# jzebedee/deltaq

Hardware: AMD Instinct MI355X
Metric: MB of text suffix-sorted per second (bit-exact SA) (higher is better)
Workload: dtype u8 text / u64 keys / int32 SA; 1 GPU; 256 MiB uniform-random bytes per GPU (splitmix64 seed 0x5EED0003+rank), int32 SA; bytes_per_gpu=268435456, residency=text and SA resident in HBM, rounds_after_initial_sort=1

## Files before the change

deltaq_amd/csrc/dq_flags.h:

```cpp
#pragma once

#include <algorithm>
#include <cstdint>
#include <cstdlib>
#include <cstring>
#include <optional>
#include <string>

namespace dq {

struct Flags {
    bool debug = false;
    std::optional<int> trace;
    std::optional<int> hip_device;
    std::optional<int> numa_bind;
    std::optional<std::string> fault;
    std::optional<int> small_n;
    std::optional<int> no_many;
    std::optional<int> mid_many_min;
    std::optional<int> no_large_many;
    std::optional<int> large_many_min;
    std::optional<int> no_diff_many;
    std::optional<int> no_diff_mid_many;
    std::optional<int> diff_mid_many_min;
    std::optional<int> no_diff_large;
    std::optional<int> diff_large_min;
    std::optional<int> diff_large_table;
    std::optional<int> no_index_many;
    std::optional<int> index_many_min;
    std::optional<int> index_many_threads;
    std::optional<int> no_index_large;
    std::optional<int> index_large_min;
    std::optional<int> no_check_many;
    std::optional<int> no_bwt_many;
    std::optional<int> no_mtf_many;
    std::optional<int> no_huff_many;
    std::optional<int> mtf_short_max;
    std::optional<int> unbz2_one_start;
    bool no_list_buffers = false;
    bool text_copy = false;
    bool assume_doubled = false;
    bool no_twins = false;
    bool no_period_hint = false;
    std::optional<int> xcd_group;
    std::optional<int> packed;
    std::optional<int> key_bytes;
    std::optional<int> coded;
    std::optional<int> split;
    bool no_bucket = false;
    std::optional<int> bucket;
    std::optional<int> bucket_keybits;
    std::optional<int> bucket_ext;
    std::optional<int> bucket_tile;
    std::optional<int> bucket_slots;
    bool old_first_pass = false;
    bool no_fused_ties = false;
    std::optional<int> sparse;
    std::optional<int> binned_isa;
    bool no_binned_isa = false;
    std::optional<int> runs;
    bool no_small = false;
    bool no_wide_small = false;
    bool no_first_small = false;
    std::optional<int> mid_groups;
    bool no_l_shift = false;
    bool no_upd_words = false;
    std::optional<int> upd_bin;
    std::optional<int> upd_bin_min;
    std::optional<int> upd_window;
    std::optional<int> chain_steps;
    bool no_chain = false;
    bool force_rshift = false;
    std::optional<int> tail_max;
    std::optional<int> pair_chains;
    std::optional<int> pair_chains_min;
    std::optional<int> pair_maxg;
    std::optional<int> late_runs_min;
    bool no_late_runs = false;
    std::optional<int> run_period;
    bool search_wave = false;
    std::optional<int> search_ptab;
    bool no_wave_windows = false;
    bool no_poll = false;
    bool no_second_stage = false;
    std::optional<int> win_min;
    std::optional<int> win_second;
    std::optional<int> walk_on;
    bool no_resume = false;
    std::optional<int> scan_device;
    std::optional<int> scan_groups;
    std::optional<int> scan_groups_cap;
    std::optional<int> scan_chains;
    std::optional<int64_t> scan_min_seg;
    std::optional<int64_t> scan_extra;
    std::optional<int64_t> scan_lane_budget;
    std::optional<int> scan_poll_sleep;
    std::optional<int> scan_spin_log2;
    std::optional<int> scan_slow_group;
    std::optional<int> scan_par_emit;
    std::optional<int64_t> frame_follow_min;
    bool frame_after = false;
};

inline Flags read_flags()
{
    auto on = [](const char *name) { return getenv(name) != nullptr; };
    auto num = [](const char *name, int lo = INT32_MIN, int hi = INT32_MAX) -> std::optional<int> {
        const char *v = getenv(name);
        if (!v) return std::nullopt;
        return std::max(lo, std::min(hi, atoi(v)));
    };
    auto num64 = [](const char *name, int64_t lo) -> std::optional<int64_t> {
        const char *v = getenv(name);
        if (!v) return std::nullopt;
        return std::max<int64_t>(lo, atoll(v));
    };
    Flags f;
    const char *gate = getenv("DQ_DEBUG_FLAGS");
    f.debug = gate && atoi(gate) != 0;
    f.trace = num("DQ_TRACE");
    f.hip_device = num("DQ_HIP_DEVICE");
    f.numa_bind = num("DQ_NUMA_BIND");
    if (!f.debug) return f;

    if (const char *v = getenv("DQ_FAULT")) f.fault = v;
    f.small_n = num("DQ_SMALL_N", 0);
    f.no_many = num("DQ_NO_MANY", 0, 15);
    f.mid_many_min = num("DQ_MID_MANY_MIN", 1);
    f.no_large_many = num("DQ_NO_LARGE_MANY", 0, 1);
    f.large_many_min = num("DQ_LARGE_MANY_MIN", 1);
    f.no_diff_many = num("DQ_NO_DIFF_MANY", 0, 1);
    f.no_diff_mid_many = num("DQ_NO_DIFF_MID_MANY", 0, 1);
    f.diff_mid_many_min = num("DQ_DIFF_MID_MANY_MIN", 1);
    f.no_diff_large = num("DQ_NO_DIFF_LARGE", 0, 1);
    f.diff_large_min = num("DQ_DIFF_LARGE_MIN", 1);
    f.diff_large_table = num("DQ_DIFF_LARGE_TABLE", 0, 1);
    f.no_index_many = num("DQ_NO_INDEX_MANY", 0, 1);
    f.index_many_min = num("DQ_INDEX_MANY_MIN", 1);
    f.index_many_threads = num("DQ_INDEX_MANY_THREADS");
    f.no_index_large = num("DQ_NO_INDEX_LARGE", 0, 1);
    f.index_large_min = num("DQ_INDEX_LARGE_MIN", 1);
    f.no_check_many = num("DQ_NO_CHECK_MANY", 0, 1);
    f.no_bwt_many = num("DQ_NO_BWT_MANY", 0, 1);
    f.no_mtf_many = num("DQ_NO_MTF_MANY", 0, 1);
    f.no_huff_many = num("DQ_NO_HUFF_MANY", 0, 1);
    f.mtf_short_max = num("DQ_MTF_SHORT_MAX", 0);
    f.unbz2_one_start = num("DQ_UNBZ2_ONE_START", 0, 1);
    f.no_list_buffers = on("DQ_NO_LIST_BUFFERS");
    f.text_copy = on("DQ_TEXT_COPY");
    f.assume_doubled = on("DQ_ASSUME_DOUBLED");
    f.no_twins = on("DQ_NO_TWINS");
    f.no_period_hint = on("DQ_NO_PERIOD_HINT");

    f.xcd_group = num("DQ_XCD_GROUP", 0, 64);
    f.packed = num("DQ_PACKED");
    f.key_bytes = num("DQ_KEY_BYTES", 1, 8);
    f.coded = num("DQ_CODED");
    f.split = num("DQ_SPLIT");
    f.no_bucket = on("DQ_NO_BUCKET");
    f.bucket = num("DQ_BUCKET");
    f.bucket_keybits = num("DQ_BUCKET_KEYBITS");
    f.bucket_ext = num("DQ_BUCKET_EXT");
    f.bucket_tile = num("DQ_BUCKET_TILE", 0, 1);
    f.bucket_slots = num("DQ_BUCKET_SLOTS", 0, 1);
    f.old_first_pass = on("DQ_OLD_FIRST_PASS");
    f.no_fused_ties = on("DQ_NO_FUSED_TIES");
    f.sparse = num("DQ_SPARSE");
    f.binned_isa = num("DQ_BINNED_ISA");
    f.no_binned_isa = on("DQ_NO_BINNED_ISA");
    f.runs = num("DQ_RUNS");

    f.no_small = on("DQ_NO_SMALL");
    f.no_wide_small = on("DQ_NO_WIDE_SMALL");
    f.no_first_small = on("DQ_NO_FIRST_SMALL");
    f.mid_groups = num("DQ_MID_GROUPS");
    f.no_l_shift = on("DQ_NO_L_SHIFT");
    f.no_upd_words = on("DQ_NO_UPD_WORDS");
    f.upd_bin = num("DQ_UPD_BIN", 0, 2);
    f.upd_bin_min = num("DQ_UPD_BIN_MIN", 1);
    f.upd_window = num("DQ_UPD_WINDOW");
    f.chain_steps = num("DQ_CHAIN_STEPS");
    f.no_chain = on("DQ_NO_CHAIN");
    f.force_rshift = on("DQ_FORCE_RSHIFT");

    f.tail_max = num("DQ_TAIL_MAX", 0);
    f.pair_chains = num("DQ_PAIR_CHAINS");
    f.pair_chains_min = num("DQ_PAIR_CHAINS_MIN", 1);
    f.pair_maxg = num("DQ_PAIR_MAXG", 2);
    f.late_runs_min = num("DQ_LATE_RUNS_MIN", 1);
    f.no_late_runs = on("DQ_NO_LATE_RUNS");
    f.run_period = num("DQ_RUN_PERIOD", 1);

    f.search_wave = on("DQ_SEARCH_WAVE");
    f.search_ptab = num("DQ_SEARCH_PTAB");
    f.no_wave_windows = on("DQ_NO_WAVE_WINDOWS");
    f.no_poll = on("DQ_NO_POLL");
    f.no_second_stage = on("DQ_NO_SECOND_STAGE");
    f.win_min = num("DQ_WIN_MIN", 16);
    f.win_second = num("DQ_WIN_SECOND", 16);
    f.walk_on = num("DQ_WALK_ON");
    f.no_resume = on("DQ_NO_RESUME");

    f.scan_device = num("DQ_SCAN_DEVICE");
    f.scan_groups = num("DQ_SCAN_GROUPS", 8);
    f.scan_groups_cap = num("DQ_SCAN_GROUPS_CAP", 0);
    f.scan_chains = num("DQ_SCAN_CHAINS", 1);
    f.scan_min_seg = num64("DQ_SCAN_MIN_SEG", 64);
    f.scan_extra = num64("DQ_SCAN_EXTRA", 1);
    f.scan_lane_budget = num64("DQ_SCAN_LANE_BUDGET", 1);
    f.scan_poll_sleep = num("DQ_SCAN_POLL_SLEEP", 1, 32);
    f.scan_spin_log2 = num("DQ_SCAN_SPIN_LOG2", 1, 24);
    f.scan_slow_group = num("DQ_SCAN_SLOW_GROUP", 0, 255);
    f.scan_par_emit = num("DQ_SCAN_PAR_EMIT");
    f.frame_follow_min = num64("DQ_FRAME_FOLLOW_MIN", INT64_MIN);
    f.frame_after = on("DQ_FRAME_AFTER");
    return f;
}

struct FaultPlan {
    int alloc_at = 0, hip_at = 0;
    int alloc_seen = 0, hip_seen = 0;
    bool spin = false;
};
inline thread_local FaultPlan t_fault;

inline FaultPlan parse_fault(const std::optional<std::string> &spec)
{
    FaultPlan p;
    if (!spec) return p;
    const char *f = spec->c_str();
    if (strncmp(f, "alloc:", 6) == 0) p.alloc_at = std::max(1, atoi(f + 6));
    else if (strncmp(f, "hip:", 4) == 0) p.hip_at = std::max(1, atoi(f + 4));
    else if (strcmp(f, "spin") == 0) p.spin = true;
    return p;
}

struct FlagState {
    Flags snap;
    int depth = 0;
};
inline thread_local FlagState t_flags;

struct EnvScope {
    EnvScope()
    {
        if (t_flags.depth++ != 0) return;
        t_flags.snap = read_flags();
        t_fault = parse_fault(t_flags.snap.fault);
    }
    explicit EnvScope(const Flags &adopt)
    {
        if (t_flags.depth++ == 0) t_flags.snap = adopt;
    }
    ~EnvScope() { if (--t_flags.depth == 0) t_fault = FaultPlan{}; }
    EnvScope(const EnvScope &) = delete;
    EnvScope &operator=(const EnvScope &) = delete;
};

inline const Flags &flags()
{
    if (t_flags.depth == 0) t_flags.snap = read_flags();
    return t_flags.snap;
}

template <typename Fn>
auto with_flags(Fn fn)
{
    return [snap = flags(), fn = std::move(fn)](auto &&...args) mutable {
        EnvScope scope(snap);
        return fn(std::forward<decltype(args)>(args)...);
    };
}

}
```

deltaq_amd/csrc/dq_round0.h:

```cpp
#pragma once
#include "dq_sort_passes.h"
#include "dq_alpha_code.h"
#include "dq_ties.h"
#include "dq_bucket_sort.h"
#include "dq_xcd_rank.h"
#include "dq_slot_rank.h"

namespace dq {
namespace {

constexpr int64_t kSgShortList = 1 << 20;
inline int mid_group_cap(int64_t list_len)
{
    if (const std::optional<int> g = flags().mid_groups) {
        return *g >= 1024 ? 1024 : *g >= 512 ? 512 : *g >= 256 ? 256 : 0;
    }
    return list_len >= kSgShortList ? 512 : 1024;
}
inline bool small_round_usable(int64_t n, int64_t mm, bool third_list_buffer)
{
    const Flags &F = flags();
    return !F.no_small && n < (1ll << 32) && (mm * 2 <= n || (third_list_buffer && !F.no_wide_small));
}

template <typename Fn>
int with_bool(bool on, Fn fn)
{
    return on ? fn(std::true_type{}) : fn(std::false_type{});
}

constexpr int kXcdHistAt = kRadixSize + 16;

template <typename IdxT>
struct Round0Out {
    uint64_t *Kr[2] = {nullptr, nullptr};
    IdxT *Vr[2] = {nullptr, nullptr};
    int64_t m = 0, h = 0;
    int rbits = 0;
    bool dense_built = false;
    bool fin_done = false;
    int64_t fin_cap = 0, fin_left = 0;
    bool shallow_ties = false, keys_ready = false, list_ungrouped = false;
    const uint32_t *first_rank32 = nullptr;
    RunPlan runs;
};

template <typename IdxT>
struct Round0 {
    DeviceCtx &c;
    hipStream_t st;
    Workspace<IdxT> &w;
    int64_t n;
    IdxT *d_sa;
    Launcher &L;
    const uint8_t *text_src;
    int period_hint;
    Round0Out<IdxT> &o;

    static constexpr int64_t wb = (int64_t)sizeof(IdxT);
    TextStats s;
    KeyPlan k;
    int ib = 0;
    bool coded = false;
    uint64_t *K[2] = {w.K0, w.K1};
    IdxT *V[2] = {nullptr, nullptr};

    const uint64_t *text64() const { return reinterpret_cast<const uint64_t *>(w.text); }
    int64_t tie_words() const { return (n + 63) / 64; }

    int digit_tables(int kb, bool coded_keys)
    {
        if (coded_keys) {
            const int hblocks = (int)std::min<int64_t>(kHistBlocks, ((n >> 2) + kHistThreads - 1) / kHistThreads + 1);
            DQ_TRY(L.begin(DQ_K_RADIX_HIST, n, n));
            HIP_TRY(hipMemsetAsync(w.hist_partial, 0, (size_t)kMaxPasses * kRadixSize * 8, st));
            hipLaunchKernelGGL(text_coded_hist_kernel, dim3(hblocks), dim3(kHistThreads), 0, st,
                               reinterpret_cast<const uint32_t *>(w.text), n, (const uint16_t *)w.codetab,
                               reinterpret_cast<unsigned long long *>(w.hist_partial));
            hipLaunchKernelGGL(radix_hist_scan_kernel, dim3(kMaxPasses), dim3(kHistScanThreads), 0, st,
                               (const unsigned long long *)w.hist_partial, w.digit_offset);
            HIP_TRY(hipGetLastError());
            return L.end();
        }
        hipLaunchKernelGGL(text_digit_offsets_kernel, dim3(kb), dim3(kBlock), 0, st,
                           (const int64_t *)w.bytehist, (const uint8_t *)w.text, n, kb, w.digit_offset);
        HIP_TRY(hipGetLastError());
        return DQ_OK;
    }

    int prepare()
    {
        int blocks = (int)std::min<int64_t>(1024, ((n >> 4) + kBlock - 1) / kBlock + 1);
        unsigned long long *xcd_hist = n >= kRound0MinN ? reinterpret_cast<unsigned long long *>(w.bytehist + kXcdHistAt) : nullptr;
        if (xcd_hist) blocks = (blocks + kXcds - 1) / kXcds * kXcds;
        HIP_TRY(hipMemsetAsync(w.bytehist, 0, (size_t)(kXcdHistAt + (xcd_hist ? kXcds * kRadixSize : 0)) * 8, L.st));
        LAUNCH(L, DQ_K_TEXT_HIST, n, n,
               hipLaunchKernelGGL(text_hist_kernel, dim3(blocks + 1), dim3(kBlock), 0, L.st,
                                  text_src ? text_src : (const uint8_t *)w.text, n, reinterpret_cast<unsigned long long *>(w.bytehist),
                                  reinterpret_cast<unsigned long long *>(w.bytehist + 256), text_src ? w.text : (uint8_t *)nullptr,
                                  xcd_hist));
        HIP_TRY(hipMemcpyAsync(c.pinned, w.bytehist, (256 + 10) * 8, hipMemcpyDeviceToHost, L.st));
        HIP_TRY(hipEventRecord(c.readback, L.st));
        constexpr int kEarlyPasses = 3;
        DQ_TRY(prepare_status<IdxT>(L, w, n, kEarlyPasses));
        if (n >= kRound0MinN) HIP_TRY(hipMemsetAsync(w.Vb, 0, (size_t)(tie_words() + 1) * 8, L.st));
        HIP_TRY(hipEventSynchronize(c.readback));
        const Flags &F = flags();
        s = TextStats(c.pinned, n);
        ib = s.ib;
        k = choose_key_bytes(s, F);
        DQ_TRY(prepare_status<IdxT>(L, w, n, k.kb, kEarlyPasses));
        bool hist_deferred = false;
        if (coded_keys_tried(s, F, k)) {
            AlphaCode code;
            if (build_alpha_code(s.hist, &code) && (code.avg_len <= kCodedMaxAvgLen || F.coded)) {
                uint16_t *stage = reinterpret_cast<uint16_t *>(c.pinned + 512);
                memcpy(stage, code.tab, sizeof(code.tab));
                HIP_TRY(hipMemcpyAsync(w.codetab, stage, sizeof(code.tab), hipMemcpyHostToDevice, L.st));
                coded = true;
                hist_deferred = split_round0_wanted(n, k, (int)wb, F);
                if (F.trace) fprintf(stderr, "[dq] coded round 0: %d symbols, %.2f bits per byte\n", code.sigma, code.avg_len);
            }
        }
        if (hist_deferred) return DQ_OK;
        return digit_tables(k.kb, coded);
    }

    int passes(int &cur, uint32_t *ebits = nullptr, uint64_t *seam_tab = nullptr)
    {
        const int kb = k.kb;
        if (k.packed) {
            DQ_TRY(rank_pass<IdxT, kTextPacked>(L, w, text64(), (const IdxT *)nullptr, K[1], (IdxT *)nullptr, n, 0, kb, ib));
            cur = 1;
            for (int p = 1; p < kb; ++p) {
                if (p == kb - 1 && ebits)
                    DQ_TRY(rank_pass<IdxT, kKeysLastTies>(L, w, K[cur], (const IdxT *)nullptr, (uint64_t *)nullptr, d_sa, n, p,
                                                          kb, ib, ebits, seam_tab));
                else if (p == kb - 1)
                    DQ_TRY(rank_pass<IdxT, kKeysLast>(L, w, K[cur], (const IdxT *)nullptr, K[cur ^ 1], d_sa, n, p, kb, ib));
                else
                    DQ_TRY(rank_pass<IdxT, kKeys>(L, w, K[cur], (const IdxT *)nullptr, K[cur ^ 1], (IdxT *)nullptr, n, p, kb, ib));
                cur ^= 1;
            }
            return DQ_OK;
        }
        DQ_TRY(with_bool(coded, [&](auto kCoded) -> int {
            return rank_pass<IdxT, kText, decltype(kCoded)::value>(L, w, text64(), (const IdxT *)nullptr, K[1], V[1], n, 0, kb);
        }));
        cur = 1;
        for (int p = 1; p < kb; ++p) {
            DQ_TRY(rank_pass<IdxT, kPairs>(L, w, K[cur], V[cur], K[cur ^ 1], V[cur ^ 1], n, p, kb));
            cur ^= 1;
        }
        return DQ_OK;
    }

    int collect_ties(uint32_t *ebits, const uint64_t *seam_tab, uint64_t *act_rank, bool *overflow, uint64_t *fin_rank,
                     bool seams = true, int64_t h_fin = -1)
    {
        using Cfg = RankCfg<IdxT, kKeysLastTies>;
        using CfgS = RankCfg<IdxT, kKeysLastTies, true>;
        const int64_t tile_keys = small_tiles(n) ? CfgS::kThreads * CfgS::kItems : Cfg::kThreads * Cfg::kItems;
        const int64_t ntiles = (n + tile_keys - 1) / tile_keys;
        const int pass = k.kb - 1;
        char *area = w.ctl_status + (size_t)pass * w.ctl_status_stride;
        const int64_t *dofs = w.digit_offset + pass * kRadixSize;
        TieCounters *ctr = reinterpret_cast<TieCounters *>(w.totals + 6);
        if (seams) {
            HIP_TRY(hipMemsetAsync(ctr, 0, sizeof(TieCounters), L.st));
            const unsigned sg = (unsigned)((ntiles * kRadixSize + kBlock - 1) / kBlock);
            DQ_TRY(with_status_word(n, [&](auto word) -> int {
                LAUNCH(L, DQ_K_TIE_SEAM, ntiles * kRadixSize, ntiles * kRadixSize * (16 + (int64_t)sizeof(uint64_t)),
                       hipLaunchKernelGGL(tie_seam_kernel<decltype(word)>, dim3(sg), dim3(kBlock), 0, L.st, seam_tab, ntiles, ib, dofs,
                                          reinterpret_cast<const decltype(word) *>(area + 256), ebits));
                return DQ_OK;
            }));
        }
        LAUNCH(L, DQ_K_TIE_COLLECT, n, n / 8,
               hipLaunchKernelGGL(tie_collect_kernel<IdxT>, dim3((unsigned)((tie_words() + kTieThreads - 1) / kTieThreads)),
                                  dim3(kTieThreads), 0, L.st, reinterpret_cast<const uint64_t *>(ebits), tie_words(), n, (const IdxT *)d_sa,
                                  act_rank, w.Va, ctr));
        unsigned long long *left_over = reinterpret_cast<unsigned long long *>(w.totals + 3);
        o.fin_cap = n / 8;
        LAUNCH(L, DQ_K_SMALL_FINISH, o.fin_cap, 0,
               hipLaunchKernelGGL((small_group_finish_kernel<IdxT, 8, 32>),
                                  dim3((unsigned)std::min<int64_t>((o.fin_cap + kFinishThreads - 1) / kFinishThreads, 256 * 16)),
                                  dim3(kFinishThreads), 0, L.st, (const uint64_t *)act_rank, (const IdxT *)w.Va, (const uint8_t *)w.text,
                                  o.fin_cap, n, h_fin >= 0 ? h_fin : (int64_t)k.kb, d_sa, fin_rank, w.Vb, left_over,
                                  (const unsigned long long *)&ctr->count));
        DQ_TRY(read_totals<IdxT>(L, c, w, 64, "radix look-back timed out (device spin bound hit)"));
        o.m = c.pinned[6];
        *overflow = c.pinned[7] != 0;
        if (*overflow && flags().trace) fprintf(stderr, "[dq] tie / bucket overflow flags: %lld\n", (long long)c.pinned[7]);
        o.fin_left = c.pinned[3];
        if (L.active && !c.pending.empty() && c.pending.back().cat == DQ_K_SMALL_FINISH) {
            const int64_t cnt = std::min<int64_t>(o.m, o.fin_cap);
            c.pending.back().elems = cnt;
            c.pending.back().bytes = cnt * (8 + wb + 64 + wb);
        }
        return DQ_OK;
    }

    int build_isa_binned(uint64_t *keys, uint64_t *P0, int kshift0)
    {
        const int64_t ntiles = (n + kSegFusedTile - 1) / kSegFusedTile;
        const size_t need = 256 + (size_t)3 * ntiles * 8;
        if (need > w.seg_status_bytes) return fail(DQ_ERR_HIP, "seg status buffer too small");
        HIP_TRY(hipMemsetAsync(w.seg_status, 0, need, st));
        const bool rank32_direct = sizeof(IdxT) == 4 && !o.runs.runs_wanted && mid_group_cap(n) > 0;
        const bool third = w.X != nullptr;
        uint32_t *list_rank = (small_round_usable(n, 0, third) && !flags().no_first_small)
                                  ? (rank32_direct ? w.RL : reinterpret_cast<uint32_t *>(w.Vb)) : nullptr;
        LAUNCH(L, DQ_K_SEG_FUSED, n, n * (8 + wb + 8),
               hipLaunchKernelGGL((seg_fused_kernel<IdxT, true, false, false, true>), dim3((unsigned)ntiles),
                                  dim3(kSegThreads), 0, st, (const uint64_t *)keys, (const IdxT *)d_sa, n, ib, kshift0,
                                  d_sa, w.ISA, P0, w.Va, reinterpret_cast<uint64_t *>(w.seg_status + 256), ntiles,
                                  reinterpret_cast<SegCtl *>(w.seg_status), w.totals, w.totals + 1, 0, list_rank, 0, spin_bound()));
        const int rc = read_totals<IdxT>(L, c, w, 16, "device look-back timed out (spin bound hit)");
        o.m = c.pinned[0];
        DQ_TRY(rc);
        DQ_TRY(isa_from_suffix_words<IdxT>(L, c, w, n, ib, k.kb, P0, keys));
        if (list_rank && o.m == 0) return DQ_OK;
        if (list_rank && small_round_usable(n, o.m, third) && rank32_direct) {
            o.first_rank32 = list_rank;
            return DQ_OK;
        }
        if (list_rank && small_round_usable(n, o.m, third)) {
            LAUNCH(L, DQ_K_KEY2_FROM_PAIRS, o.m, o.m * 12,
                   hipLaunchKernelGGL(widen_ranks_kernel, dim3(grid_for(o.m)), dim3(kBlock), 0, st,
                                      (const uint32_t *)list_rank, o.m, keys));
            return DQ_OK;
        }
        const bool with_key2 = !o.runs.runs_wanted;
        const int kbits = bit_length((uint64_t)(n - 1) + (uint64_t)k.kb);
        unsigned long long *cnt = reinterpret_cast<unsigned long long *>(w.totals + 3);
        HIP_TRY(hipMemsetAsync(cnt, 0, 8, st));
        const int64_t per = (int64_t)kPairThreads * kPairItems;
        LAUNCH(L, DQ_K_KEY2_FROM_PAIRS, n, n * 8 + o.m * (wb + 8 + wb),
               hipLaunchKernelGGL(key2_from_pairs_kernel<IdxT>, dim3((unsigned)((n + per - 1) / per)), dim3(kPairThreads),
                                  0, st, (const uint64_t *)P0, n, ib, (const IdxT *)w.ISA, (int64_t)k.kb, kbits, with_key2,
                                  keys, w.Va, cnt));
        o.keys_ready = with_key2;
        o.list_ungrouped = true;
        return DQ_OK;
    }

    int bucketed(bool *done)
    {
        *done = false;
        const Flags &F = flags();
        const BucketPlan b = plan_bucketed(s, F, k, coded, (int)wb);
        if (!b.applies) return DQ_OK;
        const int kb = k.kb, keybits = b.keybits, lowbits = b.lowbits;
        const SlotPlan sp = bucket_slots_fit(s, b, (int)wb);
        const FinishTiles ft = plan_finish_tiles(b, n, F, sp.fits);
        static_assert(sizeof(SlotRankCtl) <= (size_t)kHistBlocks * kMaxPasses * kRadixSize * 4, "the cursors live in the histogram scratch");
        const bool slots = bucket_slots_wanted(sp, ft, F) && (uint64_t)sp.words <= slot_span_words_of(w) &&
                           (size_t)(2 * kSlotBuckets + 5) * 4 <= finish_bounds_entries(n) * 8;
        uint32_t *slot_base = reinterpret_cast<uint32_t *>(w.bkt_bounds), *slot_out = slot_base + kSlotBuckets + 4;
        SlotRankCtl *sctl = reinterpret_cast<SlotRankCtl *>(w.hist_partial);
        const int first = slots ? 0 : 1;
        uint8_t *E[2] = {reinterpret_cast<uint8_t *>(w.Va), reinterpret_cast<uint8_t *>(w.Va) + align_up((size_t)n)};
        uint32_t *ebits = reinterpret_cast<uint32_t *>(w.Vb);
        TieCounters *ctr = reinterpret_cast<TieCounters *>(w.totals + 6);
        BucketFlags *bflags = reinterpret_cast<BucketFlags *>(&ctr->overflow);
        hipLaunchKernelGGL(text_digit_offsets_kernel, dim3(b.bbytes), dim3(kBlock), 0, st,
                           (const int64_t *)w.bytehist, (const uint8_t *)w.text, n, b.bbytes, w.digit_offset,
                           b.xcd_pass ? (const int64_t *)(w.bytehist + kXcdHistAt) : nullptr, b.xcd_pass ? w.xcd_offset : nullptr);
        HIP_TRY(hipGetLastError());
        if (slots) {
            if (F.trace)
                fprintf(stderr, "[dq] second pass into bucket slots: %d x %d slots of %lld words (n=%lld)\n", sp.first, sp.second,
                        (long long)b.X, (long long)n);
            HIP_TRY(hipMemsetAsync(sctl, 0, sizeof(SlotRankCtl), st));
            hipLaunchKernelGGL(slot_plan_kernel, dim3(kRadixSize + 1), dim3(kBlock), 0, st, (const int64_t *)w.bytehist, b.X, slot_base);
            HIP_TRY(hipGetLastError());
        }
        if (c.ncu <= 0) {
            int v = 0;
            c.ncu = hipDeviceGetAttribute(&v, hipDeviceAttributeMultiprocessorCount, c.dev) == hipSuccess && v > 0 ? v : 256;
        }
        if (b.xcd_pass) {
            if (F.trace) fprintf(stderr, "[dq] XCD-local first pass (n=%lld, eighths of %lld)\n", (long long)n, (long long)xcd_eighth(n));
            if (sizeof(XcdRankCtl) > w.ctl_status_stride) return fail(DQ_ERR_HIP, "status buffer too small");
            LAUNCH(L, DQ_K_RADIX_RANK, n, n * (1 + 8),
                   hipLaunchKernelGGL(xcd_text_rank_kernel, dim3((unsigned)std::min<int64_t>(c.ncu, (n + kXcdTileN - 1) / kXcdTileN)),
                                      dim3(kXcdRankThreads), 0, st, reinterpret_cast<const uint32_t *>(w.text), K[first], n,
                                      ib + lowbits, keybits, ib, (const int64_t *)w.xcd_offset,
                                      reinterpret_cast<XcdRankCtl *>(w.ctl_status)));
        } else {
            DQ_TRY(b.ext ? rank_pass_ext<IdxT, kTextPackedExt>(L, w, text64(), (const uint8_t *)nullptr, K[1], E[1], n, 0, ib, ib + lowbits, keybits)
                       : rank_pass<IdxT, kTextPacked>(L, w, text64(), (const IdxT *)nullptr, K[first], (IdxT *)nullptr, n, 0, kb, ib,
                                                      nullptr, nullptr, ib + lowbits, keybits));
        }
        if (slots) {
            const int groups = resident_groups(&c.slot_rank_groups, (const void *)slot_rank_kernel, kSlotRankThreads, c.dev);
            LAUNCH(L, DQ_K_RADIX_RANK, n, n * 16,
                   hipLaunchKernelGGL(slot_rank_kernel, dim3((unsigned)std::min<int64_t>(groups, (n + kSlotTileN - 1) / kSlotTileN)),
                                      dim3(kSlotRankThreads), 0, st, (const uint64_t *)K[0], K[1], n, ib + lowbits + 8, ib + lowbits,
                                      (const int64_t *)w.digit_offset, (const uint32_t *)slot_base, sctl, bflags));
        }
        for (int p = 1; p < b.bbytes && !slots; ++p) {
            DQ_TRY(b.ext ? rank_pass_ext<IdxT, kKeysExt>(L, w, K[p & 1], E[p & 1], K[(p & 1) ^ 1], E[(p & 1) ^ 1], n, p, ib, ib + lowbits + 8 * p, keybits)
                       : rank_pass<IdxT, kKeys>(L, w, K[p & 1], (const IdxT *)nullptr, K[(p & 1) ^ 1], (IdxT *)nullptr, n, p, kb, ib,
                                                nullptr, nullptr, ib + lowbits + 8 * p, keybits));
        }
        uint64_t *Ks = slots ? K[1] : K[b.bbytes & 1], *Kfree = slots ? K[0] : K[(b.bbytes & 1) ^ 1];
        const uint8_t *Es = b.ext ? E[b.bbytes & 1] : nullptr;
        if (F.trace)
            fprintf(stderr, "[dq] bucket finish: %s geometry, %lld tiles of up to %lld words cut every %lld %s (n=%lld)\n", ft.fine ? "fine" : "coarse",
                    (long long)ft.ntiles, (long long)ft.cap, (long long)(ft.by_id ? ft.g : ft.Cf), ft.by_id ? "buckets" : "words", (long long)n);
        if ((size_t)ft.ntiles + 1 > finish_bounds_entries(n)) return fail(DQ_ERR_HIP, "tile bounds buffer too small");
        if (slots) {
            LAUNCH(L, DQ_K_BUCKET_SORT, ft.ntiles, ft.ntiles * 16,
                   hipLaunchKernelGGL(slot_out_kernel, dim3(1), dim3(kSlotOutThreads), 0, st, sctl->cursor, (uint32_t)b.X, slot_out, bflags));
            auto kernel = bucket_sort_kernel<IdxT, false, BktFine, true>;
            const int groups = resident_groups(&c.bkt_slot_groups[sizeof(IdxT) == 8], (const void *)kernel, BktFine::threads, c.dev);
            LAUNCH(L, DQ_K_BUCKET_SORT, n, n * (8 + wb) + n / 8,
                   hipLaunchKernelGGL(kernel, dim3((unsigned)std::min<int64_t>(ft.ntiles, groups)), dim3(BktFine::threads), 0, st,
                                      (const uint64_t *)Ks, ib, lowbits, (const int64_t *)nullptr, ft.ntiles, d_sa, ebits, bflags,
                                      (const uint8_t *)nullptr, (const uint32_t *)slot_base, (const uint32_t *)sctl->cursor, (const uint32_t *)slot_out));
        } else if (ft.by_id) {
            const int64_t nbuckets = (int64_t)1 << (8 * b.bbytes);
            LAUNCH(L, DQ_K_BUCKET_SORT, ft.ntiles, ft.ntiles * 16 * 8,
                   hipLaunchKernelGGL(bucket_bounds_by_id_kernel, dim3((unsigned)((nbuckets + 1 + kBlock - 1) / kBlock)), dim3(kBlock), 0,
                                      st, (const uint64_t *)Ks, n, ib + lowbits, ft.g, b.X, nbuckets, ft.ntiles, w.bkt_bounds, bflags));
        } else {
            LAUNCH(L, DQ_K_BUCKET_SORT, ft.ntiles, ft.ntiles * 16 * 8,
                   hipLaunchKernelGGL(bucket_bounds_kernel, dim3((unsigned)((ft.ntiles + 1 + kBlock - 1) / kBlock)), dim3(kBlock), 0,
                                      st, (const uint64_t *)Ks, n, ib + lowbits, ft.Cf, b.X, ft.ntiles, w.bkt_bounds, bflags));
        }
        auto finish = [&](auto kExt, auto geometry) -> int {
            using G = decltype(geometry);
            auto kernel = bucket_sort_kernel<IdxT, decltype(kExt)::value, G>;
            const int groups = resident_groups(&c.bkt_groups[ft.fine][b.ext][sizeof(IdxT) == 8], (const void *)kernel, G::threads, c.dev);
            LAUNCH(L, DQ_K_BUCKET_SORT, n, n * ((b.ext ? 9 : 8) + wb) + n / 8,
                   hipLaunchKernelGGL(kernel, dim3((unsigned)std::min<int64_t>(ft.ntiles, groups)), dim3(G::threads), 0, st,
                                      (const uint64_t *)Ks, ib, lowbits, (const int64_t *)w.bkt_bounds, ft.ntiles, d_sa, ebits, bflags, Es,
                                      (const uint32_t *)nullptr, (const uint32_t *)nullptr, (const uint32_t *)nullptr));
            return DQ_OK;
        };
        if (slots) {
        } else if (ft.fine) {
            DQ_TRY(finish(std::false_type{}, BktFine{}));
        } else {
            DQ_TRY(with_bool(b.ext, [&](auto kExt) -> int { return finish(kExt, BktCoarse{}); }));
        }
        if (b.ext && F.trace) fprintf(stderr, "[dq] bucketed round 0 with %d + 8 key bits per suffix (n=%lld)\n", keybits, (long long)n);
        bool overflow = false;
        DQ_TRY(collect_ties(ebits, nullptr, Kfree, &overflow, Ks, false, b.hb));
        if (overflow) {
            if (F.trace) fprintf(stderr, "[dq] bucketed round 0 gave up (n=%lld): plain digit passes\n", (long long)n);
            DQ_TRY(prepare_status<IdxT>(L, w, n, kMaxPasses));
            HIP_TRY(hipMemsetAsync(w.Vb, 0, (size_t)(tie_words() + 1) * 8, st));
            HIP_TRY(hipMemsetAsync(w.totals, 0, 64, st));
            o.m = 0; o.fin_cap = 0; o.fin_left = 0;
            return digit_tables(kb, false);
        }
        o.fin_done = o.m <= o.fin_cap;
        o.Kr[0] = Kfree; o.Kr[1] = Ks;
        o.h = b.hb;
        o.shallow_ties = true;
        *done = true;
        return DQ_OK;
    }

    int split(bool *done)
    {
        *done = false;
        if constexpr (sizeof(IdxT) != 4) {
            return DQ_OK;
        } else {
            if (!w.sp_top || !w.X || !w.RL) return DQ_OK;
            const int64_t cap = std::min<int64_t>(kFinCap, (n + 2) / (kSplitBuckets / 2));
            if (cap < 2) return DQ_OK;
            const uint32_t *t32 = reinterpret_cast<const uint32_t *>(w.text);
            const uint16_t *ctab = (const uint16_t *)w.codetab;
            uint64_t *Ks[2] = {K[0], w.X};
            IdxT *Vs[2] = {w.Vb, w.Xs};
            const int64_t ovf_cap = (n / 2) & ~(int64_t)1;
            uint64_t *ovf_k[2] = {reinterpret_cast<uint64_t *>(w.ISA), K[0]};
            IdxT *ovf_v[2] = {reinterpret_cast<IdxT *>(w.RL), w.Vb};
            const Flags &F = flags();
            const bool dbg = F.trace.value_or(0) >= 2;
            auto phase = [&](const char *what) -> int {
                if (!dbg) return DQ_OK;
                HIP_TRY(hipStreamSynchronize(st));
                fprintf(stderr, "[dq] split round 0: %s done\n", what);
                return DQ_OK;
            };
            const unsigned sgrid = (unsigned)((kSplitSample + kBlock - 1) / kBlock);
            DQ_TRY(with_bool(coded, [&](auto kCoded) -> int {
                LAUNCH(L, DQ_K_SPLIT_AUX, kSplitSample, kSplitSample * ((coded ? 20 : 12) + 8),
                       hipLaunchKernelGGL(sample_keys_kernel<decltype(kCoded)::value>, dim3(sgrid), dim3(kBlock), 0, st, t32, n, ctab, kSplitSample, Ks[0]));
                return DQ_OK;
            }));
            DQ_TRY(phase("sample"));
            int scur = 0;
            DQ_TRY(onesweep_sort_pairs<IdxT>(L, w, Ks, Vs, kSplitSample, 64, scur));
            DQ_TRY(phase("sample sort"));
            HIP_TRY(hipMemsetAsync(w.sp_ctl, 0, sizeof(SplitCtl), st));
            hipLaunchKernelGGL(sample_heavy_kernel, dim3(sgrid), dim3(kBlock), 0, st, (const uint64_t *)Ks[scur], &w.sp_ctl->ovf_count);
            HIP_TRY(hipGetLastError());
            HIP_TRY(hipMemcpyAsync(c.pinned, w.sp_ctl, sizeof(SplitCtl), hipMemcpyDeviceToHost, st));
            HIP_TRY(hipStreamSynchronize(st));
            const int64_t heavy = c.pinned[0];
            if (F.trace)
                fprintf(stderr, "[dq] sample-sort round 0: %.1f %% of the sampled keys are copies of keys too heavy for a bucket%s\n",
                        100.0 * (double)heavy / (double)kSplitSample, heavy * 5 > 2 * kSplitSample ? " -- the digit passes instead" : "");
            if (heavy * 5 > 2 * kSplitSample && F.split.value_or(0) < 2) return DQ_OK;
            HIP_TRY(hipMemsetAsync(w.sp_cursor_b, 0, (size_t)kSplitBuckets * 8, st));
            HIP_TRY(hipMemsetAsync(w.sp_ctl, 0, sizeof(SplitCtl), st));
            const int64_t n_main = n & ~(int64_t)1;
            uint64_t *spill_k = reinterpret_cast<uint64_t *>(d_sa);
            IdxT *spill_v = d_sa + (n / 2 + 1);
            if (n / 8 + 1025 * (int64_t)kSplitTop + 1024 > n / 4) return DQ_OK;
            LAUNCH(L, DQ_K_SPLIT_AUX, kSplitBuckets, (int64_t)kSplitBuckets * 16,
                   hipLaunchKernelGGL(make_splitters_kernel, dim3(kSplitBuckets / kBlock), dim3(kBlock), 0, st, (const uint64_t *)Ks[scur], w.sp_top, w.sp_sub,
                                      w.sp_low, w.sp_pure);
                   hipLaunchKernelGGL(split_estimate_kernel, dim3(1), dim3(kSplitTop), 0, st, (const uint64_t *)Ks[scur], (const uint64_t *)w.sp_top, n, w.sp_off,
                                      w.sp_cursor_a));
            DQ_TRY(phase("splitters, region estimates"));
            const unsigned grid_a = (unsigned)((n + kSplitTileA - 1) / kSplitTileA);
            DQ_TRY(with_bool(coded, [&](auto kCoded) -> int {
                LAUNCH(L, DQ_K_SPLIT_PASS, n, n * (1 + 8 + wb),
                       hipLaunchKernelGGL((split_pass_kernel<IdxT, true, decltype(kCoded)::value>), dim3(grid_a), dim3(kSplitThreads), 0, st, text64(), (const IdxT *)nullptr,
                                          (const uint64_t *)nullptr, (const IdxT *)nullptr, (int64_t)0, n, (const uint64_t *)w.sp_top, w.sp_cursor_a,
                                          (const int64_t *)w.sp_off, (const unsigned long long *)nullptr, (const uint32_t *)w.sp_tile_first, K[1], w.Va, spill_k, spill_v,
                                          n_main, (uint64_t *)nullptr, (IdxT *)nullptr, (int64_t)0, w.sp_ctl, ctab));
                return DQ_OK;
            }));
            DQ_TRY(phase("pass A"));
            const unsigned grid_b = (unsigned)(n / kSplitTileB + kSplitTop);
            LAUNCH(L, DQ_K_SPLIT_PASS, n, n * 2 * (8 + wb),
                   hipLaunchKernelGGL(split_plan_kernel, dim3(1), dim3(kSplitTop), 0, st, (const unsigned long long *)w.sp_cursor_a, (const int64_t *)w.sp_off, w.sp_cnt_a,
                                      w.sp_tile_first, w.sp_ctl);
                   hipLaunchKernelGGL((split_pass_kernel<IdxT, false, false>), dim3(grid_b), dim3(kSplitThreads), 0, st, (const uint64_t *)K[1], (const IdxT *)w.Va,
                                      (const uint64_t *)spill_k, (const IdxT *)spill_v, n_main, n, (const uint64_t *)w.sp_sub, w.sp_cursor_b, (const int64_t *)w.sp_off,
                                      (const unsigned long long *)w.sp_cnt_a, (const uint32_t *)w.sp_tile_first, Ks[0], Vs[0], Ks[1], Vs[1],
                                      cap, ovf_k[0], ovf_v[0], ovf_cap, w.sp_ctl, ctab, (const uint8_t *)w.sp_pure));
            DQ_TRY(phase("pass B"));
            LAUNCH(L, DQ_K_SPLIT_AUX, kSplitBuckets, (int64_t)kSplitBuckets * 36,
                   hipLaunchKernelGGL(bucket_sum_kernel, dim3(kScanBlocks), dim3(kScanThreads), 0, st, (const unsigned long long *)w.sp_cursor_b, cap,
                                      (const uint8_t *)w.sp_pure, w.sp_part);
                   hipLaunchKernelGGL(bucket_scan_kernel, dim3(kScanBlocks), dim3(kScanThreads), 0, st, (const unsigned long long *)w.sp_cursor_b, cap,
                                      (const uint8_t *)w.sp_pure, (const ScanPart *)w.sp_part, w.sp_out_base, w.sp_ovf_src, w.sp_ovf_dst, w.sp_ctl));
            DQ_TRY(phase("bucket scan"));
            const bool two = cap > kFinSmallCap;
            LAUNCH(L, DQ_K_SPLIT_FINISH, n, n * 2 * (8 + wb),
                   if (two || cap <= kFinSmallCap)
                       hipLaunchKernelGGL((bucket_finish_kernel<IdxT, 256, 4>), dim3(kSplitBuckets), dim3(256), 0, st, (const uint64_t *)Ks[0], (const IdxT *)Vs[0],
                                          (const uint64_t *)Ks[1], (const IdxT *)Vs[1], cap, (int64_t)0, (int64_t)kFinSmallCap, !two,
                                          (const unsigned long long *)w.sp_cursor_b, (const int64_t *)w.sp_out_base, K[1], d_sa, ovf_k[0], ovf_v[0], ovf_cap, w.sp_ctl, (const uint8_t *)w.sp_pure);
                   if (cap > kFinSmallCap)
                       hipLaunchKernelGGL((bucket_finish_kernel<IdxT, 256, 8>), dim3(kSplitBuckets), dim3(256), 0, st, (const uint64_t *)Ks[0], (const IdxT *)Vs[0],
                                          (const uint64_t *)Ks[1], (const IdxT *)Vs[1], cap, (int64_t)(two ? kFinSmallCap : 0), (int64_t)kFinCap, true,
                                          (const unsigned long long *)w.sp_cursor_b, (const int64_t *)w.sp_out_base, K[1], d_sa, ovf_k[0], ovf_v[0], ovf_cap, w.sp_ctl, (const uint8_t *)w.sp_pure));
            HIP_TRY(hipMemcpyAsync(c.pinned, w.sp_ctl, sizeof(SplitCtl), hipMemcpyDeviceToHost, st));
            HIP_TRY(hipStreamSynchronize(st));
            const int64_t ovf = c.pinned[0], ovf_buckets = c.pinned[1], npure = c.pinned[4];
            const bool abandon = c.pinned[3] != 0 || ovf + npure > ovf_cap;
            if (flags().trace)
                fprintf(stderr, "[dq] sample-sort round 0 (%s keys, %d buckets of <= %lld): %lld suffixes in %lld oversize buckets, %lld copies of heavy keys placed unsorted%s\n",
                        coded ? "coded" : "raw", kSplitBuckets, (long long)cap, (long long)ovf, (long long)ovf_buckets, (long long)npure,
                        abandon ? " -- overflow lists full, given up" : "");
            if (abandon) return DQ_OK;
            if (npure > 0) {
                LAUNCH(L, DQ_K_SPLIT_AUX, npure, npure * 2 * (8 + wb),
                       hipLaunchKernelGGL(pure_place_kernel<IdxT>, dim3((unsigned)((npure + kBlock - 1) / kBlock)), dim3(kBlock), 0, st, npure, ovf_cap,
                                          (const uint64_t *)ovf_k[0], (const IdxT *)ovf_v[0], (const int64_t *)w.sp_out_base, (const uint64_t *)w.sp_low, K[1], d_sa));
            }
            if (ovf > 0) {
                int xcur = 0;
                DQ_TRY(onesweep_sort_pairs<IdxT>(L, w, ovf_k, ovf_v, ovf, 64, xcur));
                LAUNCH(L, DQ_K_SPLIT_AUX, ovf, ovf * 2 * (8 + wb),
                       hipLaunchKernelGGL(overflow_place_kernel<IdxT>, dim3((unsigned)((ovf + kBlock - 1) / kBlock)), dim3(kBlock), 0, st, ovf, ovf_buckets,
                                          (const int64_t *)w.sp_ovf_src, (const int64_t *)w.sp_ovf_dst,
                                          (const uint64_t *)ovf_k[xcur], (const IdxT *)ovf_v[xcur], K[1], d_sa));
            }
            *done = true;
            return DQ_OK;
        }
    }

    int run()
    {
        const Flags &F = flags();
        int cur = 0;
        DQ_TRY(prepare());
        const int kb = k.kb;
        o.runs = plan_runs(s, F, (int)wb, period_hint);
        V[kb & 1] = d_sa;
        V[(kb & 1) ^ 1] = w.Va;
        o.Vr[0] = w.Va; o.Vr[1] = w.Vb;
        o.rbits = ib;
        o.h = kb;
        bool done = false;
        DQ_TRY(bucketed(&done));
        if (done) return DQ_OK;
        if (fused_ties_wanted(n, k, F)) {
            uint32_t *ebits = reinterpret_cast<uint32_t *>(w.Vb);
            uint64_t *seam_tab = reinterpret_cast<uint64_t *>(reinterpret_cast<char *>(w.Vb) +
                                                              align_up((size_t)(tie_words() + 1) * 8));
            DQ_TRY(passes(cur, ebits, seam_tab));
            bool overflow = false;
            DQ_TRY(collect_ties(ebits, seam_tab, K[cur], &overflow, K[cur ^ 1]));
            o.fin_done = !overflow && o.m <= o.fin_cap;
            if (!overflow) {
                o.Kr[0] = K[cur]; o.Kr[1] = K[cur ^ 1];
                return DQ_OK;
            }
            HIP_TRY(hipMemsetAsync(w.ctl_status + (size_t)(kb - 1) * w.ctl_status_stride, 0, w.ctl_status_stride, st));
            DQ_TRY(rank_pass<IdxT, kKeysLast>(L, w, K[cur ^ 1], (const IdxT *)nullptr, K[cur], d_sa, n, kb - 1, kb, ib));
        } else {
            bool split_done = false;
            const bool split_wanted = split_round0_wanted(n, k, (int)wb, F);
            if (split_wanted && (!o.runs.runs_wanted || F.split)) {
                DQ_TRY(split(&split_done));
            }
            if (split_wanted && !split_done) {
                DQ_TRY(digit_tables(kb, coded));
                DQ_TRY(prepare_status<IdxT>(L, w, n, kb));
            }
            if (split_done) {
                cur = 1;
            } else {
                DQ_TRY(passes(cur));
            }
        }
        const int kshift0 = k.packed ? ib : 0;
        const DenseGuess guess = dense_guess(n, k);
        int64_t tied_pairs = 0;
        if (guess == DenseGuess::kTakeSample) {
            HIP_TRY(hipMemsetAsync(w.totals + 2, 0, 8, st));
            hipLaunchKernelGGL(sample_ties_kernel, dim3(kTieSamples / kBlock), dim3(kBlock), 0, st,
                               (const uint64_t *)K[cur], n, kshift0, kTieSamples, w.totals + 2);
            HIP_TRY(hipGetLastError());
            HIP_TRY(hipMemcpyAsync(c.pinned, w.totals + 2, 8, hipMemcpyDeviceToHost, st));
            HIP_TRY(hipStreamSynchronize(st));
            tied_pairs = c.pinned[0];
        }
        o.dense_built = predict_dense(guess, tied_pairs, F);
        if (o.dense_built && binned_isa_pays(n, F)) {
            o.Kr[0] = K[cur]; o.Kr[1] = K[cur ^ 1];
            return build_isa_binned(K[cur], K[cur ^ 1], kshift0);
        }
        o.Kr[0] = K[cur ^ 1]; o.Kr[1] = K[cur];
        return o.dense_built ? rebucket<IdxT, true, false, true>(L, c, w, K[cur], (const IdxT *)d_sa, n, 0, kshift0, d_sa, o.Kr[0], w.Va, &o.m)
                             : rebucket<IdxT, true, false, false>(L, c, w, K[cur], (const IdxT *)d_sa, n, 0, kshift0, d_sa, o.Kr[0], w.Va, &o.m);
    }
};

}
}
```

deltaq_amd/csrc/dq_round0_plan.h:

```cpp
#pragma once
#include <algorithm>
#include <cmath>
#include <cstddef>
#include <cstdint>

#include "dq_flags.h"

namespace dq {

constexpr int kKgramSamples = 1024;
constexpr int kBktCap = 12288;
constexpr int kBktCapFine = 6144;
constexpr int kSplitTop = 512;
constexpr int kSplitSub = 512;
constexpr int kSplitBuckets = kSplitTop * kSplitSub;
constexpr int kFinCap = 2048;
constexpr int64_t kSplitMinN = 5ll << 20;
constexpr int64_t kCodedMinN = 8ll << 20;
constexpr double kCodedMaxAvgLen = 5.8;
constexpr int kTieSamples = 4096;
constexpr int64_t kRound0MinN = 1 << 16;

inline int index_bits(int64_t n) { return n <= 1 ? 1 : 64 - __builtin_clzll((uint64_t)(n - 1)); }

struct TextStats {
    int64_t n = 0;
    int ib = 1;
    int64_t hist[256] = {};
    int64_t kgram[8] = {};
    bool long_run = false;
    int64_t run_chunks = 0;
    double h0 = 0;
    int sigma = 0;
    int64_t cmax = 0;

    TextStats() = default;
    TextStats(const int64_t *words, int64_t n_) : n(n_), ib(index_bits(n_)), long_run(words[256 + 8] != 0), run_chunks(words[256 + 9])
    {
        std::copy(words, words + 256, hist);
        std::copy(words + 256, words + 256 + 8, kgram);
        for (int b = 0; b < 256; ++b) {
            cmax = std::max(cmax, hist[b]);
            if (hist[b] > 0) { ++sigma; const double p = (double)hist[b] / (double)n; h0 -= p * std::log2(p); }
        }
    }
};

struct KeyPlan { int kb = 8; bool packed = false; };

inline KeyPlan choose_key_bytes(const TextStats &s, const Flags &F)
{
    const int64_t n = s.n;
    const double need = std::log2((double)std::max<int64_t>(n, 2)) + 10.0;
    int kb = 8;
    if (s.h0 >= 0.25) kb = std::min(8, std::max(3, (int)std::ceil(need / s.h0)));
    const int fit = (64 - s.ib) / 8;
    bool packed = fit >= 2 && (kb <= fit || (double)fit * s.h0 >= std::log2((double)std::max<int64_t>(n, 2)) + 3.0);
    if (n >= kKgramSamples * 8) {
        const int L = packed ? std::min(kb, fit) : kb;
        const int64_t C = s.kgram[std::max(L, 1) - 1];
        const double twins = (double)n * 2.0 * (double)C / ((double)kKgramSamples * (double)kKgramSamples);
        if (C >= kKgramSamples / 16 && twins > 0.25) { packed = false; kb = 8; }
    }
    if (F.packed) packed = *F.packed != 0 && fit >= 2;
    if (packed) kb = std::min(kb, fit);
    if (F.key_bytes) {
        kb = *F.key_bytes;
        if (kb > fit || kb < 2) packed = false;
    }
    return {kb, packed};
}

inline bool coded_keys_tried(const TextStats &s, const Flags &F, KeyPlan k)
{
    bool coded = !k.packed && k.kb == 8 && s.n >= kCodedMinN;
    if (coded) coded = s.h0 <= kCodedMaxAvgLen - 0.25 && (s.sigma <= 128 || s.n >= 2 * kCodedMinN);
    if (F.coded) coded = *F.coded != 0 && !k.packed && k.kb == 8 && s.n >= 64;
    return coded;
}

inline bool split_round0_wanted(int64_t n, KeyPlan k, int idx_bytes, const Flags &F)
{
    if (idx_bytes != 4 || k.packed || k.kb != 8 || n < kSplitMinN || n > (int64_t)kSplitBuckets * (kFinCap / 2)) return false;
    if (F.split) return *F.split != 0;
    if (F.key_bytes || F.no_bucket) return false;
    return n >= (64ll << 20);
}

struct BucketPlan {
    bool applies = false;
    int keybits = 0, bbytes = 0, lowbits = 0;
    int64_t X = 0, C = 0, ntiles = 0;
    bool ext = false;
    bool xcd_pass = false;
    int64_t hb = 0;
};

inline BucketPlan plan_bucketed(const TextStats &s, const Flags &F, KeyPlan k, bool coded, int idx_bytes)
{
    const int64_t n = s.n;
    const int ib = s.ib;
    BucketPlan p;
    if (coded) return p;
    if (F.no_bucket || F.no_fused_ties || F.sparse || F.key_bytes) return p;
    const bool forced = F.bucket.has_value();
    if (ib > 31 || n < kRound0MinN) return p;
    if (!forced && s.long_run) return p;
    int keybits = std::min(64 - ib, 36);
    if (F.bucket_keybits) keybits = std::max(17, std::min(keybits, *F.bucket_keybits));
    const double tied = (double)n * std::exp2(-(double)keybits * s.h0 / 8.0);
    if (!k.packed) {
        if (!forced && (k.kb >= 8 || tied > 0.3)) return p;
    }
    const double pm = (double)s.cmax / (double)n;
    int bbytes = 2;
    double est = (double)n * pm * pm;
    double need = est + 6.0 * std::sqrt(est) + 64.0;
    const bool force3 = forced && *F.bucket == 3;
    if (need > 5120 || (!forced && n < (12 << 20)) || force3) {
        if (keybits - 24 >= 8 && (forced || n >= (12 << 20))) {
            bbytes = 3;
            est *= pm;
            need = est + 6.0 * std::sqrt(est) + 64.0;
        }
        if (need > 5120 || (bbytes == 2 && !forced)) {
            if (!forced) return p;
            need = 5120;
        }
    }
    p.applies = true;
    p.keybits = keybits;
    p.bbytes = bbytes;
    p.X = std::min<int64_t>(((int64_t)need + 255) / 256 * 256, 5120);
    p.C = kBktCap - p.X;
    p.lowbits = keybits - 8 * bbytes;
    p.ntiles = (n + p.C - 1) / p.C;
    const bool room = (size_t)2 * (((size_t)n + 255) / 256 * 256) <= (size_t)(n + 2) * (size_t)idx_bytes;
    p.ext = keybits + 8 <= 56 && p.lowbits + 8 <= 18 && tied > 0.02 && room;
    if (F.bucket_ext) p.ext = *F.bucket_ext != 0 && keybits + 8 <= 56 && room;
    p.xcd_pass = !p.ext && !F.old_first_pass;
    p.hb = (keybits + (p.ext ? 8 : 0)) / 8;
    return p;
}

constexpr int64_t kBktFineMinN = 12ll << 20;
struct FinishTiles {
    bool fine = false;
    bool by_id = false;
    int64_t cap = 0;
    int64_t Cf = 0, g = 0;
    int64_t ntiles = 0;
};

inline FinishTiles plan_finish_tiles(const BucketPlan &b, int64_t n, const Flags &F, bool slots_fit = false)
{
    FinishTiles t;
    if (!b.applies) return t;
    const bool can = b.bbytes == 2 && !b.ext;
    t.fine = can && (F.bucket_tile ? *F.bucket_tile != 0 : !F.bucket.has_value() && n >= kBktFineMinN);
    t.cap = t.fine ? kBktCapFine : kBktCap;
    const int64_t Cf = t.cap - b.X;
    const bool force_by_id = t.fine && slots_fit && F.bucket_slots && *F.bucket_slots == 1;
    if (force_by_id) {
        t.by_id = true;
        t.g = 1;
        t.ntiles = (int64_t)1 << (8 * b.bbytes);
    } else if (Cf >= b.X) {
        t.Cf = Cf;
        t.ntiles = (n + Cf - 1) / Cf;
    } else {
        t.by_id = true;
        t.g = std::min<int64_t>(t.cap / b.X, 64);
        const int64_t nbuckets = (int64_t)1 << (8 * b.bbytes);
        t.ntiles = (nbuckets + t.g - 1) / t.g;
    }
    return t;
}

inline int64_t slot_span_words(int64_t n, int idx_bytes) { return (n + 2) * (int64_t)(8 + idx_bytes) / 8; }

struct SlotPlan {
    bool fits = false;
    int first = 0, second = 0;
    int64_t words = 0;
};

inline SlotPlan bucket_slots_fit(const TextStats &s, const BucketPlan &b, int idx_bytes)
{
    SlotPlan p;
    if (!b.applies || b.bbytes != 2 || b.ext) return p;
    p.first = s.sigma;
    p.second = s.sigma + (s.hist[0] == 0 ? 1 : 0);
    p.words = (int64_t)p.first * p.second * b.X;
    p.fits = p.words <= slot_span_words(s.n, idx_bytes) && p.words < ((int64_t)1 << 32);
    return p;
}

inline void slot_bases(const int64_t *hist , int64_t X, uint32_t *base )
{
    int ra[257], rb[257];
    ra[0] = rb[0] = 0;
    for (int d = 0; d < 256; ++d) {
        ra[d + 1] = ra[d] + (hist[d] > 0 ? 1 : 0);
        rb[d + 1] = rb[d] + (hist[d] > 0 || d == 0 ? 1 : 0);
    }
    for (int A = 0; A < 256; ++A)
        for (int B = 0; B < 256; ++B)
            base[A * 256 + B] = (uint32_t)(X * ((int64_t)ra[A] * rb[256] + (hist[A] > 0 ? rb[B] : 0)));
    base[65536] = (uint32_t)(X * ra[256] * rb[256]);
}

inline bool bucket_slots_wanted(const SlotPlan &p, const FinishTiles &t, const Flags &F)
{
    if (F.bucket_slots && *F.bucket_slots == 0) return false;
    return p.fits && t.fine && t.by_id && t.g == 1;
}

inline size_t finish_bounds_entries(int64_t n)
{
    const size_t by_words = (size_t)n / (kBktCapFine / 2) + 4;
    return n < kRound0MinN ? by_words : std::max<size_t>(by_words, 65536 + 4);
}

inline bool fused_ties_wanted(int64_t n, KeyPlan k, const Flags &F)
{
    return k.packed && k.kb >= 2 && n >= kRound0MinN && !F.no_fused_ties && !F.sparse;
}

enum class DenseGuess { kNeither, kGuessDense, kTakeSample };

inline DenseGuess dense_guess(int64_t n, KeyPlan k)
{
    if (n < kRound0MinN || k.packed || k.kb != 8) return DenseGuess::kNeither;
    return n < (8 << 20) ? DenseGuess::kGuessDense : DenseGuess::kTakeSample;
}

inline bool predict_dense(DenseGuess g, int64_t tied_pairs, const Flags &F)
{
    if (F.sparse) return *F.sparse == 0;
    return g == DenseGuess::kGuessDense || (g == DenseGuess::kTakeSample && tied_pairs * 12 > kTieSamples);
}

inline bool binned_isa_pays(int64_t n, const Flags &F)
{
    const bool pays = F.binned_isa ? *F.binned_isa != 0 : n > (32ll << 20);
    return pays && n >= kRound0MinN && 2 * index_bits(n) <= 63 && !F.no_binned_isa;
}

struct RunPlan {
    bool runs_wanted = false;
    bool long_run_seen = false;
    bool late_runs_possible = false;
};

inline RunPlan plan_runs(const TextStats &s, const Flags &F, int idx_bytes, int period_hint)
{
    RunPlan r;
    const bool can = idx_bytes == 4 && s.n >= kRound0MinN;
    r.long_run_seen = can && s.long_run;
    r.runs_wanted = (r.long_run_seen && s.run_chunks * 16 * 16 >= s.n) || (period_hint > 0 && can);
    r.late_runs_possible = can;
    if (F.runs) { r.runs_wanted = idx_bytes == 4 && *F.runs != 0; r.late_runs_possible = r.late_runs_possible && *F.runs != 0; }
    if (F.mid_groups) r.runs_wanted = r.runs_wanted && *F.mid_groups >= 256;
    return r;
}

}
```

deltaq_amd/csrc/dq_sa_kernels.h:

```cpp
#pragma once
#include "dq_runs.h"
#include "dq_device_utils.h"

namespace dq {

template <typename IdxT>
__global__ __launch_bounds__(kBlock) void gather_key2_kernel(uint64_t *__restrict__ comp,
                                                             const IdxT *__restrict__ suf,
                                                             const IdxT *__restrict__ ISA,
                                                             int64_t m, int64_t n, int64_t h, int kbits,
                                                             int rshift = 0,
                                                             const uint32_t *__restrict__ RL = nullptr ,
                                                             const uint8_t *__restrict__ text = nullptr, int run_order = 0)
{
    for (int64_t j = (int64_t)blockIdx.x * kBlock + threadIdx.x; j < m;
         j += (int64_t)gridDim.x * kBlock) {
        const int64_t s = (int64_t)suf[j];
        int64_t off = h;
        uint64_t k2 = 0;
        bool keyed = false;
        if (RL) {
            const uint32_t r = RL[s];
            if (run_order) { k2 = (int64_t)r >= h ? (uint64_t)run_order_key(text, n, s, r, run_order) : 0ull; keyed = true; }
            else if ((int64_t)r > h) off = (int64_t)r;
        }
        if (!keyed) {
            const int64_t q = s + off;
            k2 = q < n ? (uint64_t)((int64_t)ISA[q] + h) : (off > h ? 0ull : (uint64_t)(n - 1 - s));
        }
        comp[j] = ((comp[j] >> rshift) << kbits) | k2;
    }
}

static __global__ __launch_bounds__(kBlock) void keys_to_ranks_kernel(uint64_t *__restrict__ comp, int64_t m, int kbits)
{
    for (int64_t j = (int64_t)blockIdx.x * kBlock + threadIdx.x; j < m; j += (int64_t)gridDim.x * kBlock)
        comp[j] >>= kbits;
}

template <typename IdxT>
__global__ __launch_bounds__(kBlock) void gather_text_key_kernel(uint64_t *__restrict__ comp,
                                                                 const IdxT *__restrict__ suf,
                                                                 const uint8_t *__restrict__ text,
                                                                 int64_t m, int64_t n, int64_t h, int ebytes)
{
    const int kbits = 8 * ebytes + 3;
    for (int64_t j = (int64_t)blockIdx.x * kBlock + threadIdx.x; j < m;
         j += (int64_t)gridDim.x * kBlock) {
        const int64_t q = (int64_t)suf[j] + h;
        int64_t len = n - q;
        len = len < 0 ? 0 : (len > ebytes ? ebytes : len);
        uint64_t bytes = 0;
        for (int b = 0; b < ebytes; ++b) bytes = (bytes << 8) | (b < len ? (uint64_t)text[q + b] : 0ull);
        comp[j] = (comp[j] << kbits) | (bytes << 3) | (uint64_t)len;
    }
}

constexpr int kFinishThreads = 256;

template <typename IdxT, int kMaxG, int kMaxLen>
__global__ __launch_bounds__(kFinishThreads) void small_group_finish_kernel(
    const uint64_t *__restrict__ rank, const IdxT *__restrict__ suf, const uint8_t *__restrict__ text,
    int64_t m, int64_t n, int64_t h, IdxT *__restrict__ SA, uint64_t *__restrict__ out_rank,
    IdxT *__restrict__ out_suf, unsigned long long *__restrict__ out_count,
    const unsigned long long *__restrict__ m_dev = nullptr)
{
    if (m_dev) {
        const unsigned long long real = m_dev[0];
        if (real > (unsigned long long)m || m_dev[1] != 0) return;
        m = (int64_t)real;
    }
    __shared__ uint32_t wave_tot[kFinishThreads / kWave];
    __shared__ unsigned long long s_base;
    const int lane = lane_id();
    const int w = threadIdx.x >> 6;
    for (int64_t j0 = (int64_t)blockIdx.x * kFinishThreads; j0 < m; j0 += (int64_t)gridDim.x * kFinishThreads) {
    const int64_t j = j0 + threadIdx.x;

    uint32_t emit = 0;
    uint64_t r = 0;
    int g = 1;
    bool head = false;
    if (j < m) {
        r = rank[j];
        int left = 0, right = 0;
#pragma unroll
        for (int i = 1; i <= kMaxG; ++i)
            if (left == i - 1 && j - i >= 0 && rank[j - i] == r) left = i;
#pragma unroll
        for (int i = 1; i <= kMaxG; ++i)
            if (right == i - 1 && j + i < m && rank[j + i] == r) right = i;
        g = left + right + 1;
        if (g > kMaxG) emit = 1;
        else head = left == 0;
    }
    int64_t s[kMaxG];
    if (head) {
#pragma unroll
        for (int i = 0; i < kMaxG; ++i) s[i] = i < g ? (int64_t)suf[j + i] : 0;
        static_assert(kMaxLen % 8 == 0, "whole words");
        typedef uint64_t u64_any __attribute__((aligned(1)));
        auto cmp = [&](int64_t a, int64_t b) -> int {
            const int64_t pa = a + h, pb = b + h;
            uint64_t wa[kMaxLen / 8], wbv[kMaxLen / 8];
#pragma unroll
            for (int k = 0; k < kMaxLen / 8; ++k) {
                wa[k] = *reinterpret_cast<const u64_any *>(text + pa + 8 * k);
                wbv[k] = *reinterpret_cast<const u64_any *>(text + pb + 8 * k);
            }
            int d = kMaxLen;
            bool a_less = false;
#pragma unroll
            for (int k = kMaxLen / 8 - 1; k >= 0; --k) {
                const uint64_t x = __builtin_bswap64(wa[k]), y = __builtin_bswap64(wbv[k]);
                if (x != y) { d = 8 * k + (__builtin_clzll(x ^ y) >> 3); a_less = x < y; }
            }
            const int64_t la = n - pa, lb = n - pb;
            const int64_t lim = la < lb ? (la < kMaxLen ? la : kMaxLen) : (lb < kMaxLen ? lb : kMaxLen);
            if (d < lim) return a_less ? -1 : 1;
            if (lim < kMaxLen) return la < lb ? -1 : 1;
            return 0;
        };
        bool decided = true;
        if (g == 2) {
            const int c = cmp(s[0], s[1]);
            if (c == 0) decided = false;
            if (c > 0) { const int64_t t = s[0]; s[0] = s[1]; s[1] = t; }
        } else
#pragma unroll
        for (int pass = 0; pass < kMaxG - 1; ++pass) {
#pragma unroll
            for (int i = 0; i < kMaxG - 1; ++i) {
                if (i + 1 < g && i < g - 1 - pass) {
                    const int c = cmp(s[i], s[i + 1]);
                    if (c == 0) decided = false;
                    if (c > 0) { const int64_t t = s[i]; s[i] = s[i + 1]; s[i + 1] = t; }
                }
            }
        }
        if (decided) {
#pragma unroll
            for (int i = 0; i < kMaxG; ++i)
                if (i < g) SA[(int64_t)r + i] = (IdxT)s[i];
        } else {
            emit = (uint32_t)g;
        }
    }
    const uint32_t incl = wave_incl_sum(emit);
    if (lane == kWave - 1) wave_tot[w] = incl;
    __syncthreads();
    uint32_t off = incl - emit, tot = 0;
#pragma unroll
    for (int k = 0; k < kFinishThreads / kWave; ++k) {
        const uint32_t c = wave_tot[k];
        if (k < w) off += c;
        tot += c;
    }
    if (threadIdx.x == 0) s_base = tot ? atomicAdd(out_count, (unsigned long long)tot) : 0ull;
    __syncthreads();
    if (emit != 0) {
        const int64_t o = (int64_t)s_base + off;
        if (head) {
            for (int i = 0; i < g; ++i) { out_rank[o + i] = r; out_suf[o + i] = suf[j + i]; }
        } else {
            out_rank[o] = r;
            out_suf[o] = suf[j];
        }
    }
    __syncthreads();
    }
}

static __global__ __launch_bounds__(kBlock) void sample_ties_kernel(const uint64_t *__restrict__ keys, int64_t m,
                                                             int kshift, int samples, int64_t *__restrict__ count)
{
    const int i = blockIdx.x * kBlock + threadIdx.x;
    bool tie = false;
    if (i < samples && m > 1) {
        const int64_t p = (int64_t)((__int128)i * (m - 1) / samples);
        tie = (keys[p] >> kshift) == (keys[p + 1] >> kshift);
    }
    const uint64_t b = __ballot(tie);
    if (lane_id() == 0 && b) atomicAdd((unsigned long long *)count, (unsigned long long)__popcll(b));
}

template <typename IdxT>
__global__ __launch_bounds__(kBlock) void isa_from_sa_kernel(const IdxT *__restrict__ SA,
                                                             IdxT *__restrict__ ISA, int64_t n)
{
    for (int64_t p = (int64_t)blockIdx.x * kBlock + threadIdx.x; p < n; p += (int64_t)gridDim.x * kBlock)
        ISA[SA[p]] = (IdxT)p;
}

template <typename IdxT>
__global__ __launch_bounds__(kBlock) void sa_words_kernel(const IdxT *__restrict__ SA, int64_t n, int ib,
                                                          uint64_t *__restrict__ words)
{
    for (int64_t p = (int64_t)blockIdx.x * kBlock + threadIdx.x; p < n; p += (int64_t)gridDim.x * kBlock)
        words[p] = ((uint64_t)p << ib) | (uint64_t)SA[p];
}

template <typename IdxT>
__global__ __launch_bounds__(kBlock) void isa_scatter_kernel(const uint64_t *__restrict__ rank,
                                                             const IdxT *__restrict__ suf,
                                                             IdxT *__restrict__ ISA, int64_t m)
{
    for (int64_t j = (int64_t)blockIdx.x * kBlock + threadIdx.x; j < m; j += (int64_t)gridDim.x * kBlock)
        ISA[suf[j]] = (IdxT)rank[j];
}

}
```

deltaq_amd/csrc/dq_slot_rank.h:

```cpp
#pragma once
#include "dq_bucket_sort.h"
#include "dq_xcd_rank.h"

namespace dq {

constexpr int kSlotBuckets = 1 << 16;

struct SlotRankCtl {
    uint32_t ticket[kXcds];
    uint32_t pad[64 - kXcds];
    uint32_t cursor[kSlotBuckets];
};

static __global__ __launch_bounds__(kBlock) void slot_plan_kernel(const int64_t *__restrict__ bytehist, int64_t X,
                                                           uint32_t *__restrict__ slot_base )
{
    __shared__ int tmp[kWavesPerBlock];
    __shared__ int s_rank, s_present;
    const int d = threadIdx.x, A = blockIdx.x;
    const int pa = bytehist[d] > 0 ? 1 : 0, pb = (pa || d == 0) ? 1 : 0;
    int na, nb;
    const int ra = block_excl_sum(pa, tmp, &na);
    __syncthreads();
    const int rb = block_excl_sum(pb, tmp, &nb);
    if (A == kRadixSize) {
        if (d == 0) slot_base[kSlotBuckets] = (uint32_t)(X * na * nb);
        return;
    }
    if (d == A) { s_rank = ra; s_present = pa; }
    __syncthreads();
    slot_base[A * kRadixSize + d] = (uint32_t)(X * ((int64_t)s_rank * nb + (s_present ? rb : 0)));
}

constexpr int kSlotOutThreads = 1024;
static __global__ __launch_bounds__(kSlotOutThreads) void slot_out_kernel(uint32_t *__restrict__ count , uint32_t X,
                                                                   uint32_t *__restrict__ out ,
                                                                   BucketFlags *__restrict__ flags)
{
    constexpr int kPer = kSlotBuckets / kSlotOutThreads, kVec = kPer / 4;
    __shared__ uint32_t wtot[kSlotOutThreads / kWave];
    const int tid = threadIdx.x, lane = lane_id(), wv = tid >> 6;
    uint4 *cv = reinterpret_cast<uint4 *>(count) + tid * kVec;
    uint4 c[kVec];
#pragma unroll
    for (int i = 0; i < kVec; ++i) c[i] = cv[i];
    uint32_t sum = 0, mx = 0;
#pragma unroll
    for (int i = 0; i < kVec; ++i) {
        mx = max(max(max(c[i].x, c[i].y), max(c[i].z, c[i].w)), mx);
        c[i].x = min(c[i].x, X); c[i].y = min(c[i].y, X); c[i].z = min(c[i].z, X); c[i].w = min(c[i].w, X);
        sum += c[i].x + c[i].y + c[i].z + c[i].w;
    }
    if (mx > X) {
        atomicOr(&flags->overflow, 2ull);
#pragma unroll
        for (int i = 0; i < kVec; ++i) cv[i] = c[i];
    }
    const uint32_t incl = wave_incl_sum(sum);
    if (lane == kWave - 1) wtot[wv] = incl;
    __syncthreads();
    uint32_t run = incl - sum;
    for (int i = 0; i < wv; ++i) run += wtot[i];
    uint4 *ov = reinterpret_cast<uint4 *>(out) + tid * kVec;
#pragma unroll
    for (int i = 0; i < kVec; ++i) {
        uint4 o;
        o.x = run; run += c[i].x;
        o.y = run; run += c[i].y;
        o.z = run; run += c[i].z;
        o.w = run; run += c[i].w;
        ov[i] = o;
    }
    if (tid == kSlotOutThreads - 1) out[kSlotBuckets] = run;
}

#ifdef DQ_SLOT_PHASE_TIMING
__device__ long long *g_slot_ts = nullptr;
__device__ unsigned int g_slot_ts_next = 0;
#define DQ_SLOT_PHASE(i) do { if (threadIdx.x == 0 && g_slot_ts) g_slot_ts[(long long)ts_row * 8 + (i)] = clock64(); } while (0)
#else
#define DQ_SLOT_PHASE(i) do { } while (0)
#endif

constexpr int kSlotRankThreads = 1024;
constexpr int kSlotRankItems = 12;
constexpr int kSlotTileN = kSlotRankThreads * kSlotRankItems;

static __global__ __launch_bounds__(kSlotRankThreads, 1) void slot_rank_kernel(
    const uint64_t *__restrict__ kin , uint64_t *__restrict__ wout, int64_t n,
    int shift , int bshift ,
    const int64_t *__restrict__ region , const uint32_t *__restrict__ slot_base ,
    SlotRankCtl *__restrict__ ctl, BucketFlags *__restrict__ flags)
{
    constexpr int kThreads = kSlotRankThreads, kItems = kSlotRankItems, kTileN = kSlotTileN;
    constexpr int kPerXcd = kRadixSize / kXcds;
    __shared__ __attribute__((aligned(16))) uint64_t exch[kTileN];
    __shared__ uint32_t cnt[kRadixSize];
    __shared__ uint32_t tile_base[kRadixSize];
    __shared__ uint32_t gofs[kRadixSize];
    __shared__ uint32_t glim[kRadixSize];
    __shared__ uint32_t wtmp[kRadixSize / kWave];
    __shared__ uint32_t r_lo[kRadixSize], r_hi[kRadixSize], r_tiles[kRadixSize];
    __shared__ uint32_t xs[kXcds][kPerXcd + 1];
    __shared__ uint32_t s_lo, s_cnt;

    const int tid = threadIdx.x;
    const int w = tid >> 6;
    const int lane = lane_id();
    const uint32_t xcd = hw_xcc_id();

    if (tid < kRadixSize) {
        const int64_t lo = region[tid], hi = tid + 1 < kRadixSize ? region[tid + 1] : n;
        r_lo[tid] = (uint32_t)lo;
        r_hi[tid] = (uint32_t)hi;
        r_tiles[tid] = (uint32_t)((hi - lo + kTileN - 1) / kTileN);
        cnt[tid] = 0;
    }
    __syncthreads();
    if (tid < kXcds) {
        uint32_t run = 0;
        for (int j = 0; j < kPerXcd; ++j) { xs[tid][j] = run; run += r_tiles[tid + kXcds * j]; }
        xs[tid][kPerXcd] = run;
    }
    __syncthreads();

    int tried = 0;
    int32_t pend_e = -1;
    uint32_t pend_t = 0;
    auto issue = [&]() {
        pend_e = -1;
        for (; tried < kXcds; ++tried) {
            const int32_t e = (int32_t)((xcd + (uint32_t)tried) & (kXcds - 1));
            if (xs[e][kPerXcd] > 0) { pend_e = e; pend_t = atomicAdd(&ctl->ticket[e], 1u); return; }
        }
    };
    auto resolve = [&]() {
        while (pend_e >= 0) {
            if (pend_t < xs[pend_e][kPerXcd]) {
                int j = 0;
                while (xs[pend_e][j + 1] <= pend_t) ++j;
                const int B = pend_e + kXcds * j;
                const uint32_t lo = r_lo[B] + (pend_t - xs[pend_e][j]) * (uint32_t)kTileN;
                const uint32_t left = r_hi[B] - lo;
                s_lo = lo;
                s_cnt = left < (uint32_t)kTileN ? left : (uint32_t)kTileN;
                return;
            }
            ++tried;
            issue();
        }
        s_cnt = 0;
    };

    if (tid == 0) { issue(); resolve(); issue(); }
    __syncthreads();
    uint32_t lo = s_lo, valid = s_cnt;

    uint64_t nw[kItems];
    auto load_words = [&](uint32_t at, uint32_t m) {
        if (m == 0) return;
        const uint64_t *src = kin + at;
#pragma unroll
        for (int k = 0; k < kItems; ++k) {
            const uint32_t q = (uint32_t)(k * kThreads + tid);
            nw[k] = src[q < m ? q : m - 1];
        }
    };
    load_words(lo, valid);
#ifdef DQ_SLOT_PHASE_TIMING
    __shared__ uint32_t s_row;
#endif

    while (valid > 0) {
#ifdef DQ_SLOT_PHASE_TIMING
        if (tid == 0) s_row = g_slot_ts ? atomicAdd(&g_slot_ts_next, 1u) : 0u;
#endif
        uint64_t key[kItems];
#pragma unroll
        for (int k = 0; k < kItems; ++k) key[k] = nw[k];
        const uint32_t B = digit_of(key[0], bshift);
        uint32_t sbase = 0, room = 0;
        if (tid < kRadixSize) {
            const uint32_t b = (uint32_t)tid * kRadixSize + B;
            sbase = slot_base[b];
            room = slot_base[b + 1] - sbase;
        }
        if (tid == 0) { resolve(); issue(); }
        __syncthreads();
#ifdef DQ_SLOT_PHASE_TIMING
        const uint32_t ts_row = s_row;
#endif
        DQ_SLOT_PHASE(0);
        const uint32_t next_lo = s_lo, next_valid = s_cnt;
        load_words(next_lo, next_valid);

        uint32_t pos[kItems];
#pragma unroll
        for (int k = 0; k < kItems; ++k)
            pos[k] = atomicAdd(&cnt[digit_of(key[k], shift)], (uint32_t)(k * kThreads + tid) < valid ? 1u : 0u);
        __syncthreads();
        DQ_SLOT_PHASE(1);

        uint32_t tot = 0, incl = 0, abase = 0;
        if (tid < kRadixSize) {
            tot = cnt[tid];
            cnt[tid] = 0;
            if (tot && room) abase = atomicAdd(&ctl->cursor[(uint32_t)tid * kRadixSize + B], tot);
            incl = wave_incl_sum(tot);
            if (lane == kWave - 1) wtmp[w] = incl;
        }
        __syncthreads();
        uint32_t excl_tile = 0;
        if (tid < kRadixSize) {
            uint32_t off = 0;
#pragma unroll
            for (int i = 0; i < kRadixSize / kWave; ++i) if (i < w) off += wtmp[i];
            excl_tile = off + incl - tot;
            tile_base[tid] = excl_tile;
        }
        __syncthreads();

#pragma unroll
        for (int k = 0; k < kItems; ++k)
            if ((uint32_t)(k * kThreads + tid) < valid) exch[pos[k] + tile_base[digit_of(key[k], shift)]] = key[k];
        if (tid < kRadixSize) {
            gofs[tid] = sbase + abase - excl_tile;
            glim[tid] = excl_tile + (abase < room ? room - abase : 0u);
            if (tot && abase + tot > room) atomicOr(&flags->overflow, 2ull);
        }
        __syncthreads();
        DQ_SLOT_PHASE(2);
#pragma unroll
        for (int k = 0; k < kItems; ++k) key[k] = exch[k * kThreads + tid];

#pragma unroll
        for (int k = 0; k < kItems; ++k) {
            const uint32_t q = (uint32_t)(k * kThreads + tid);
            const uint32_t d = digit_of(key[k], shift);
            if (q < valid && q < glim[d]) wout[gofs[d] + q] = key[k];
        }
        DQ_SLOT_PHASE(3);
        lo = next_lo;
        valid = next_valid;
    }
}

}
```

deltaq_amd/csrc/dq_ties.h:

```cpp
#pragma once
#include "dq_onesweep.h"

namespace dq {

constexpr int kTieMaxRun = 4096;
constexpr int kTieThreads = 1024;

template <typename StatusT>
__global__ __launch_bounds__(kBlock) void tie_seam_kernel(const uint64_t *__restrict__ seam_tab, int64_t ntiles,
                                                          int ib, const int64_t *__restrict__ digit_offset,
                                                          const StatusT *__restrict__ status,
                                                          uint32_t *__restrict__ ebits)
{
    using SB = StatusBits<StatusT>;
    const int64_t idx = (int64_t)blockIdx.x * kBlock + threadIdx.x;
    if (idx >= ntiles * kRadixSize) return;
    const int64_t t = idx / kRadixSize;
    const int d = (int)(idx % kRadixSize);
    const uint64_t first = seam_tab[idx * 2];
    if (first == kSeamEmpty || t == 0) return;
    int64_t tp = t - 1;
    while (tp >= 0 && seam_tab[(tp * kRadixSize + d) * 2] == kSeamEmpty) --tp;
    if (tp < 0) return;
    const uint64_t last = seam_tab[(tp * kRadixSize + d) * 2 + 1];
    if ((last >> ib) != (first >> ib)) return;
    const int64_t o = digit_offset[d] + (int64_t)(status[(t - 1) * kRadixSize + d] & SB::kMask);
    atomicOr(&ebits[(uint64_t)o >> 5], 1u << ((uint32_t)o & 31u));
}

struct TieCounters {
    unsigned long long count;
    unsigned long long overflow;
};

template <typename IdxT>
__global__ __launch_bounds__(kTieThreads) void tie_collect_kernel(const uint64_t *__restrict__ ebits, int64_t nwords,
                                                                  int64_t n, const IdxT *__restrict__ SA,
                                                                  uint64_t *__restrict__ act_rank,
                                                                  IdxT *__restrict__ act_suf,
                                                                  TieCounters *__restrict__ ctr)
{
    __shared__ uint32_t wave_tot[kTieThreads / kWave];
    __shared__ unsigned long long s_base;
    const int lane = lane_id();
    const int w = threadIdx.x >> 6;
    const int64_t i = (int64_t)blockIdx.x * kTieThreads + threadIdx.x;

    uint64_t E = 0, own = 0;
    uint32_t tail = 0;
    bool over = false;
    if (i < nwords) {
        E = ebits[i];
        const uint64_t next0 = (i + 1 < nwords) ? (ebits[i + 1] & 1ull) : 0ull;
        const uint64_t A = E | (E >> 1) | (next0 << 63);
        const int lead = (E & 1ull) ? (E == ~0ull ? 64 : __builtin_ctzll(~E)) : 0;
        own = lead >= 64 ? 0ull : (A & (~0ull << lead));
        if (own >> 63 && next0) {
            int64_t j = i + 1;
            for (;;) {
                const uint64_t F = j < nwords ? ebits[j] : 0ull;
                const int c = F == ~0ull ? 64 : __builtin_ctzll(~F);
                tail += (uint32_t)c;
                if (c < 64) break;
                if (tail > (uint32_t)kTieMaxRun) { over = true; break; }
                ++j;
            }
        }
    }
    if (over) { atomicExch(&ctr->overflow, 1ull); tail = 0; own = 0; }
    const uint32_t cnt = (uint32_t)__popcll(own) + tail;
    const uint32_t incl = wave_incl_sum(cnt);
    if (lane == kWave - 1) wave_tot[w] = incl;
    __syncthreads();
    uint32_t off = incl - cnt, tot = 0;
#pragma unroll
    for (int k = 0; k < kTieThreads / kWave; ++k) {
        const uint32_t c = wave_tot[k];
        if (k < w) off += c;
        tot += c;
    }
    if (threadIdx.x == 0) s_base = tot ? atomicAdd(&ctr->count, (unsigned long long)tot) : 0ull;
    __syncthreads();
    const int64_t out = (int64_t)s_base + off;
    const uint32_t wave_members = __shfl(incl, kWave - 1, kWave);
    if (wave_members < 512u) {
        int64_t o = out, head = 0;
        uint64_t rest = own;
        while (rest) {
            const int b = __builtin_ctzll(rest);
            rest &= rest - 1;
            const int64_t p = i * 64 + b;
            if (!((E >> b) & 1ull)) head = p;
            act_rank[o] = (uint64_t)head;
            act_suf[o] = SA[p];
            ++o;
        }
        for (uint32_t k = 0; k < tail; ++k) {
            act_rank[o] = (uint64_t)head;
            act_suf[o] = SA[(i + 1) * 64 + k];
            ++o;
        }
        return;
    }
    uint64_t todo = __ballot(cnt != 0);
    const uint64_t lbit = 1ull << lane;
    while (todo) {
        const int j = __builtin_ctzll(todo);
        todo &= todo - 1;
        const uint64_t own_j = ((uint64_t)(uint32_t)__builtin_amdgcn_readlane((int)(uint32_t)(own >> 32), j) << 32) |
                               (uint32_t)__builtin_amdgcn_readlane((int)(uint32_t)own, j);
        const uint64_t E_j = ((uint64_t)(uint32_t)__builtin_amdgcn_readlane((int)(uint32_t)(E >> 32), j) << 32) |
                             (uint32_t)__builtin_amdgcn_readlane((int)(uint32_t)E, j);
        const int64_t out_j = (int64_t)(((uint64_t)(uint32_t)__builtin_amdgcn_readlane((int)(uint32_t)((uint64_t)out >> 32), j) << 32) |
                                        (uint32_t)__builtin_amdgcn_readlane((int)(uint32_t)(uint64_t)out, j));
        const uint32_t tail_j = (uint32_t)__builtin_amdgcn_readlane((int)tail, j);
        const int64_t p0 = (i - lane + j) * 64;
        if (own_j & lbit) {
            const uint64_t below = lbit - 1;
            const int64_t p = p0 + lane;
            const int64_t head = (E_j & lbit) ? p0 + (63 - __builtin_clzll(~E_j & below)) : p;
            const int64_t o = out_j + __popcll(own_j & below);
            act_rank[o] = (uint64_t)head;
            act_suf[o] = SA[p];
        }
        if (tail_j) {
            const int64_t head = p0 + (63 - __builtin_clzll(~E_j));
            const int64_t o0 = out_j + __popcll(own_j);
            for (uint32_t k = (uint32_t)lane; k < tail_j; k += kWave) {
                act_rank[o0 + k] = (uint64_t)head;
                act_suf[o0 + k] = SA[p0 + 64 + k];
            }
        }
    }
    (void)n;
}

}
```

Before: 91850 MB/s.

## Fuse tie collection with small-group settling and parallelize slot prefix kernel

Adds a tie_settle kernel that, when fine finish tiles are in use, scans tie bitmaps per tile, queues small tie groups in shared memory and sorts them in place by direct text comparison. Only the unresolved or large groups are written to the active rank/suffix lists, which replaces the separate collect plus small-group-finish launches and the full list round trip. The slot_out kernel now runs across several workgroups instead of one, and bucket planning plus the control-block memset are hoisted into prepare so digit tables are skipped when bucketing applies. The cost is more complex control flow with block-wide queue rounds, atomics, and a changed output buffer mapping for later rounds.

Result: no change. 91850 MB/s (-0.0%).

```diff
diff --git a/deltaq_amd/csrc/dq_flags.h b/deltaq_amd/csrc/dq_flags.h
--- a/deltaq_amd/csrc/dq_flags.h
+++ b/deltaq_amd/csrc/dq_flags.h
@@ -53,6 +53,7 @@
     std::optional<int> bucket_ext;
     std::optional<int> bucket_tile;
     std::optional<int> bucket_slots;
+    std::optional<int> tie_settle;
     bool old_first_pass = false;
     bool no_fused_ties = false;
     std::optional<int> sparse;
@@ -163,6 +164,7 @@
     f.bucket_ext = num("DQ_BUCKET_EXT");
     f.bucket_tile = num("DQ_BUCKET_TILE", 0, 1);
     f.bucket_slots = num("DQ_BUCKET_SLOTS", 0, 1);
+    f.tie_settle = num("DQ_TIE_SETTLE", 0, 1);
     f.old_first_pass = on("DQ_OLD_FIRST_PASS");
     f.no_fused_ties = on("DQ_NO_FUSED_TIES");
     f.sparse = num("DQ_SPARSE");
diff --git a/deltaq_amd/csrc/dq_round0.h b/deltaq_amd/csrc/dq_round0.h
--- a/deltaq_amd/csrc/dq_round0.h
+++ b/deltaq_amd/csrc/dq_round0.h
@@ -62,6 +62,10 @@
     KeyPlan k;
     int ib = 0;
     bool coded = false;
+    BucketPlan bplan;
+    SlotPlan splan;
+    FinishTiles ftiles;
+    bool slots = false;
     uint64_t *K[2] = {w.K0, w.K1};
     IdxT *V[2] = {nullptr, nullptr};
 
@@ -103,7 +107,10 @@
         HIP_TRY(hipEventRecord(c.readback, L.st));
         constexpr int kEarlyPasses = 3;
         DQ_TRY(prepare_status<IdxT>(L, w, n, kEarlyPasses));
-        if (n >= kRound0MinN) HIP_TRY(hipMemsetAsync(w.Vb, 0, (size_t)(tie_words() + 1) * 8, L.st));
+        if (n >= kRound0MinN) {
+            HIP_TRY(hipMemsetAsync(w.Vb, 0, (size_t)(tie_words() + 1) * 8, L.st));
+            HIP_TRY(hipMemsetAsync(w.hist_partial, 0, sizeof(SlotRankCtl), L.st));
+        }
         HIP_TRY(hipEventSynchronize(c.readback));
         const Flags &F = flags();
         s = TextStats(c.pinned, n);
@@ -122,7 +129,12 @@
                 if (F.trace) fprintf(stderr, "[dq] coded round 0: %d symbols, %.2f bits per byte\n", code.sigma, code.avg_len);
             }
         }
-        if (hist_deferred) return DQ_OK;
+        bplan = plan_bucketed(s, F, k, coded, (int)wb);
+        splan = bucket_slots_fit(s, bplan, (int)wb);
+        ftiles = plan_finish_tiles(bplan, n, F, splan.fits);
+        slots = bucket_slots_wanted(splan, ftiles, F) && (uint64_t)splan.words <= slot_span_words_of(w) &&
+                (size_t)(2 * kSlotBuckets + 5) * 4 <= finish_bounds_entries(n) * 8;
+        if (hist_deferred || bplan.applies) return DQ_OK;
         return digit_tables(k.kb, coded);
     }
 
@@ -156,7 +168,7 @@
     }
 
     int collect_ties(uint32_t *ebits, const uint64_t *seam_tab, uint64_t *act_rank, bool *overflow, uint64_t *fin_rank,
-                     bool seams = true, int64_t h_fin = -1)
+                     bool seams = true, int64_t h_fin = -1, bool settle = false)
     {
         using Cfg = RankCfg<IdxT, kKeysLastTies>;
         using CfgS = RankCfg<IdxT, kKeysLastTies, true>;
@@ -176,18 +188,27 @@
                 return DQ_OK;
             }));
         }
-        LAUNCH(L, DQ_K_TIE_COLLECT, n, n / 8,
-               hipLaunchKernelGGL(tie_collect_kernel<IdxT>, dim3((unsigned)((tie_words() + kTieThreads - 1) / kTieThreads)),
-                                  dim3(kTieThreads), 0, L.st, reinterpret_cast<const uint64_t *>(ebits), tie_words(), n, (const IdxT *)d_sa,
-                                  act_rank, w.Va, ctr));
         unsigned long long *left_over = reinterpret_cast<unsigned long long *>(w.totals + 3);
-        o.fin_cap = n / 8;
-        LAUNCH(L, DQ_K_SMALL_FINISH, o.fin_cap, 0,
-               hipLaunchKernelGGL((small_group_finish_kernel<IdxT, 8, 32>),
-                                  dim3((unsigned)std::min<int64_t>((o.fin_cap + kFinishThreads - 1) / kFinishThreads, 256 * 16)),
-                                  dim3(kFinishThreads), 0, L.st, (const uint64_t *)act_rank, (const IdxT *)w.Va, (const uint8_t *)w.text,
-                                  o.fin_cap, n, h_fin >= 0 ? h_fin : (int64_t)k.kb, d_sa, fin_rank, w.Vb, left_over,
-                                  (const unsigned long long *)&ctr->count));
+        const int64_t h_cmp = h_fin >= 0 ? h_fin : (int64_t)k.kb;
+        if (settle) {
+            o.fin_cap = n;
+            LAUNCH(L, DQ_K_TIE_COLLECT, n, n / 8,
+                   hipLaunchKernelGGL(tie_settle_kernel<IdxT>, dim3(tie_settle_grid(tie_words())), dim3(kSettleThreads), 0, L.st,
+                                      reinterpret_cast<const uint64_t *>(ebits), tie_words(), n, d_sa, (const uint8_t *)w.text, h_cmp,
+                                      act_rank, w.Va, left_over, ctr));
+        } else {
+            LAUNCH(L, DQ_K_TIE_COLLECT, n, n / 8,
+                   hipLaunchKernelGGL(tie_collect_kernel<IdxT>, dim3((unsigned)((tie_words() + kTieThreads - 1) / kTieThreads)),
+                                      dim3(kTieThreads), 0, L.st, reinterpret_cast<const uint64_t *>(ebits), tie_words(), n, (const IdxT *)d_sa,
+                                      act_rank, w.Va, ctr));
+            o.fin_cap = n / 8;
+            LAUNCH(L, DQ_K_SMALL_FINISH, o.fin_cap, 0,
+                   hipLaunchKernelGGL((small_group_finish_kernel<IdxT, 8, 32>),
+                                      dim3((unsigned)std::min<int64_t>((o.fin_cap + kFinishThreads - 1) / kFinishThreads, 256 * 16)),
+                                      dim3(kFinishThreads), 0, L.st, (const uint64_t *)act_rank, (const IdxT *)w.Va, (const uint8_t *)w.text,
+                                      o.fin_cap, n, h_cmp, d_sa, fin_rank, w.Vb, left_over,
+                                      (const unsigned long long *)&ctr->count));
+        }
         DQ_TRY(read_totals<IdxT>(L, c, w, 64, "radix look-back timed out (device spin bound hit)"));
         o.m = c.pinned[6];
         *overflow = c.pinned[7] != 0;
@@ -198,6 +219,8 @@
             c.pending.back().elems = cnt;
             c.pending.back().bytes = cnt * (8 + wb + 64 + wb);
         }
+        if (L.active && settle && !c.pending.empty() && c.pending.back().cat == DQ_K_TIE_COLLECT)
+            c.pending.back().bytes = n / 8 + o.m * (wb + 64 + wb);
         return DQ_OK;
     }
 
@@ -249,14 +272,12 @@
     {
         *done = false;
         const Flags &F = flags();
-        const BucketPlan b = plan_bucketed(s, F, k, coded, (int)wb);
+        const BucketPlan &b = bplan;
         if (!b.applies) return DQ_OK;
         const int kb = k.kb, keybits = b.keybits, lowbits = b.lowbits;
-        const SlotPlan sp = bucket_slots_fit(s, b, (int)wb);
-        const FinishTiles ft = plan_finish_tiles(b, n, F, sp.fits);
+        const SlotPlan &sp = splan;
+        const FinishTiles &ft = ftiles;
         static_assert(sizeof(SlotRankCtl) <= (size_t)kHistBlocks * kMaxPasses * kRadixSize * 4, "the cursors live in the histogram scratch");
-        const bool slots = bucket_slots_wanted(sp, ft, F) && (uint64_t)sp.words <= slot_span_words_of(w) &&
-                           (size_t)(2 * kSlotBuckets + 5) * 4 <= finish_bounds_entries(n) * 8;
         uint32_t *slot_base = reinterpret_cast<uint32_t *>(w.bkt_bounds), *slot_out = slot_base + kSlotBuckets + 4;
         SlotRankCtl *sctl = reinterpret_cast<SlotRankCtl *>(w.hist_partial);
         const int first = slots ? 0 : 1;
@@ -272,7 +293,6 @@
             if (F.trace)
                 fprintf(stderr, "[dq] second pass into bucket slots: %d x %d slots of %lld words (n=%lld)\n", sp.first, sp.second,
                         (long long)b.X, (long long)n);
-            HIP_TRY(hipMemsetAsync(sctl, 0, sizeof(SlotRankCtl), st));
             hipLaunchKernelGGL(slot_plan_kernel, dim3(kRadixSize + 1), dim3(kBlock), 0, st, (const int64_t *)w.bytehist, b.X, slot_base);
             HIP_TRY(hipGetLastError());
         }
@@ -313,7 +333,7 @@
         if ((size_t)ft.ntiles + 1 > finish_bounds_entries(n)) return fail(DQ_ERR_HIP, "tile bounds buffer too small");
         if (slots) {
             LAUNCH(L, DQ_K_BUCKET_SORT, ft.ntiles, ft.ntiles * 16,
-                   hipLaunchKernelGGL(slot_out_kernel, dim3(1), dim3(kSlotOutThreads), 0, st, sctl->cursor, (uint32_t)b.X, slot_out, bflags));
+                   hipLaunchKernelGGL(slot_out_kernel, dim3(kSlotOutGroups), dim3(kSlotOutThreads), 0, st, sctl->cursor, (uint32_t)b.X, slot_out, bflags));
             auto kernel = bucket_sort_kernel<IdxT, false, BktFine, true>;
             const int groups = resident_groups(&c.bkt_slot_groups[sizeof(IdxT) == 8], (const void *)kernel, BktFine::threads, c.dev);
             LAUNCH(L, DQ_K_BUCKET_SORT, n, n * (8 + wb) + n / 8,
@@ -348,7 +368,8 @@
         }
         if (b.ext && F.trace) fprintf(stderr, "[dq] bucketed round 0 with %d + 8 key bits per suffix (n=%lld)\n", keybits, (long long)n);
         bool overflow = false;
-        DQ_TRY(collect_ties(ebits, nullptr, Kfree, &overflow, Ks, false, b.hb));
+        const bool settle = tie_settle_wanted(b, ft, F);
+        DQ_TRY(collect_ties(ebits, nullptr, Kfree, &overflow, Ks, false, b.hb, settle));
         if (overflow) {
             if (F.trace) fprintf(stderr, "[dq] bucketed round 0 gave up (n=%lld): plain digit passes\n", (long long)n);
             DQ_TRY(prepare_status<IdxT>(L, w, n, kMaxPasses));
@@ -359,6 +380,11 @@
         }
         o.fin_done = o.m <= o.fin_cap;
         o.Kr[0] = Kfree; o.Kr[1] = Ks;
+        if (settle) {
+            o.fin_done = true;
+            o.Kr[0] = Ks; o.Vr[0] = w.Vb;
+            o.Kr[1] = Kfree; o.Vr[1] = w.Va;
+        }
         o.h = b.hb;
         o.shallow_ties = true;
         *done = true;
diff --git a/deltaq_amd/csrc/dq_round0_plan.h b/deltaq_amd/csrc/dq_round0_plan.h
--- a/deltaq_amd/csrc/dq_round0_plan.h
+++ b/deltaq_amd/csrc/dq_round0_plan.h
@@ -216,6 +216,13 @@
     return p.fits && t.fine && t.by_id && t.g == 1;
 }
 
+inline bool tie_settle_wanted(const BucketPlan &b, const FinishTiles &t, const Flags &F)
+{
+    if (!b.applies) return false;
+    if (F.tie_settle) return *F.tie_settle != 0;
+    return t.fine;
+}
+
 inline size_t finish_bounds_entries(int64_t n)
 {
     const size_t by_words = (size_t)n / (kBktCapFine / 2) + 4;
diff --git a/deltaq_amd/csrc/dq_sa_kernels.h b/deltaq_amd/csrc/dq_sa_kernels.h
--- a/deltaq_amd/csrc/dq_sa_kernels.h
+++ b/deltaq_amd/csrc/dq_sa_kernels.h
@@ -58,6 +58,56 @@
 
 constexpr int kFinishThreads = 256;
 
+template <int kMaxLen>
+__device__ inline int suffix_window_cmp(const uint8_t *__restrict__ text, int64_t n, int64_t h, int64_t a, int64_t b)
+{
+    static_assert(kMaxLen % 8 == 0, "whole words");
+    typedef uint64_t u64_any __attribute__((aligned(1)));
+    const int64_t pa = a + h, pb = b + h;
+    uint64_t wa[kMaxLen / 8], wbv[kMaxLen / 8];
+#pragma unroll
+    for (int k = 0; k < kMaxLen / 8; ++k) {
+        wa[k] = *reinterpret_cast<const u64_any *>(text + pa + 8 * k);
+        wbv[k] = *reinterpret_cast<const u64_any *>(text + pb + 8 * k);
+    }
+    int d = kMaxLen;
+    bool a_less = false;
+#pragma unroll
+    for (int k = kMaxLen / 8 - 1; k >= 0; --k) {
+        const uint64_t x = __builtin_bswap64(wa[k]), y = __builtin_bswap64(wbv[k]);
+        if (x != y) { d = 8 * k + (__builtin_clzll(x ^ y) >> 3); a_less = x < y; }
+    }
+    const int64_t la = n - pa, lb = n - pb;
+    const int64_t lim = la < lb ? (la < kMaxLen ? la : kMaxLen) : (lb < kMaxLen ? lb : kMaxLen);
+    if (d < lim) return a_less ? -1 : 1;
+    if (lim < kMaxLen) return la < lb ? -1 : 1;
+    return 0;
+}
+
+template <int kMaxG, int kMaxLen>
+__device__ __forceinline__ bool sort_tie_group(int64_t (&s)[kMaxG], int g, const uint8_t *__restrict__ text, int64_t n, int64_t h)
+{
+    bool decided = true;
+    if (g == 2) {
+        const int c = suffix_window_cmp<kMaxLen>(text, n, h, s[0], s[1]);
+        if (c == 0) decided = false;
+        if (c > 0) { const int64_t t = s[0]; s[0] = s[1]; s[1] = t; }
+        return decided;
+    }
+#pragma unroll
+    for (int pass = 0; pass < kMaxG - 1; ++pass) {
+#pragma unroll
+        for (int i = 0; i < kMaxG - 1; ++i) {
+            if (i + 1 < g && i < g - 1 - pass) {
+                const int c = suffix_window_cmp<kMaxLen>(text, n, h, s[i], s[i + 1]);
+                if (c == 0) decided = false;
+                if (c > 0) { const int64_t t = s[i]; s[i] = s[i + 1]; s[i + 1] = t; }
+            }
+        }
+    }
+    return decided;
+}
+
 template <typename IdxT, int kMaxG, int kMaxLen>
 __global__ __launch_bounds__(kFinishThreads) void small_group_finish_kernel(
     const uint64_t *__restrict__ rank, const IdxT *__restrict__ suf, const uint8_t *__restrict__ text,
@@ -98,47 +148,7 @@
     if (head) {
 #pragma unroll
         for (int i = 0; i < kMaxG; ++i) s[i] = i < g ? (int64_t)suf[j + i] : 0;
-        static_assert(kMaxLen % 8 == 0, "whole words");
-        typedef uint64_t u64_any __attribute__((aligned(1)));
-        auto cmp = [&](int64_t a, int64_t b) -> int {
-            const int64_t pa = a + h, pb = b + h;
-            uint64_t wa[kMaxLen / 8], wbv[kMaxLen / 8];
-#pragma unroll
-            for (int k = 0; k < kMaxLen / 8; ++k) {
-                wa[k] = *reinterpret_cast<const u64_any *>(text + pa + 8 * k);
-                wbv[k] = *reinterpret_cast<const u64_any *>(text + pb + 8 * k);
-            }
-            int d = kMaxLen;
-            bool a_less = false;
-#pragma unroll
-            for (int k = kMaxLen / 8 - 1; k >= 0; --k) {
-                const uint64_t x = __builtin_bswap64(wa[k]), y = __builtin_bswap64(wbv[k]);
-                if (x != y) { d = 8 * k + (__builtin_clzll(x ^ y) >> 3); a_less = x < y; }
-            }
-            const int64_t la = n - pa, lb = n - pb;
-            const int64_t lim = la < lb ? (la < kMaxLen ? la : kMaxLen) : (lb < kMaxLen ? lb : kMaxLen);
-            if (d < lim) return a_less ? -1 : 1;
-            if (lim < kMaxLen) return la < lb ? -1 : 1;
-            return 0;
-        };
-        bool decided = true;
-        if (g == 2) {
-            const int c = cmp(s[0], s[1]);
-            if (c == 0) decided = false;
-            if (c > 0) { const int64_t t = s[0]; s[0] = s[1]; s[1] = t; }
-        } else
-#pragma unroll
-        for (int pass = 0; pass < kMaxG - 1; ++pass) {
-#pragma unroll
-            for (int i = 0; i < kMaxG - 1; ++i) {
-                if (i + 1 < g && i < g - 1 - pass) {
-                    const int c = cmp(s[i], s[i + 1]);
-                    if (c == 0) decided = false;
-                    if (c > 0) { const int64_t t = s[i]; s[i] = s[i + 1]; s[i + 1] = t; }
-                }
-            }
-        }
-        if (decided) {
+        if (sort_tie_group<kMaxG, kMaxLen>(s, g, text, n, h)) {
 #pragma unroll
             for (int i = 0; i < kMaxG; ++i)
                 if (i < g) SA[(int64_t)r + i] = (IdxT)s[i];
diff --git a/deltaq_amd/csrc/dq_slot_rank.h b/deltaq_amd/csrc/dq_slot_rank.h
--- a/deltaq_amd/csrc/dq_slot_rank.h
+++ b/deltaq_amd/csrc/dq_slot_rank.h
@@ -33,45 +33,45 @@
 }
 
 constexpr int kSlotOutThreads = 1024;
-static __global__ __launch_bounds__(kSlotOutThreads) void slot_out_kernel(uint32_t *__restrict__ count , uint32_t X,
+constexpr int kSlotOutGroups = kSlotBuckets / kSlotOutThreads;
+static __global__ __launch_bounds__(kSlotOutThreads) void slot_out_kernel(uint32_t *count , uint32_t X,
                                                                    uint32_t *__restrict__ out ,
                                                                    BucketFlags *__restrict__ flags)
 {
-    constexpr int kPer = kSlotBuckets / kSlotOutThreads, kVec = kPer / 4;
-    __shared__ uint32_t wtot[kSlotOutThreads / kWave];
+    constexpr int kVecMax = (kSlotBuckets - kSlotOutThreads) / 4 / kSlotOutThreads + 1;
+    __shared__ uint32_t wtot[kSlotOutThreads / kWave], wfront[kSlotOutThreads / kWave];
     const int tid = threadIdx.x, lane = lane_id(), wv = tid >> 6;
-    uint4 *cv = reinterpret_cast<uint4 *>(count) + tid * kVec;
-    uint4 c[kVec];
-#pragma unroll
-    for (int i = 0; i < kVec; ++i) c[i] = cv[i];
-    uint32_t sum = 0, mx = 0;
-#pragma unroll
-    for (int i = 0; i < kVec; ++i) {
-        mx = max(max(max(c[i].x, c[i].y), max(c[i].z, c[i].w)), mx);
-        c[i].x = min(c[i].x, X); c[i].y = min(c[i].y, X); c[i].z = min(c[i].z, X); c[i].w = min(c[i].w, X);
-        sum += c[i].x + c[i].y + c[i].z + c[i].w;
-    }
-    if (mx > X) {
+    const int j = blockIdx.x;
+    const int b = j * kSlotOutThreads + tid;
+    const int nvec = j * (kSlotOutThreads / 4);
+    const uint4 *cv = reinterpret_cast<const uint4 *>(count);
+    uint4 c[kVecMax];
+#pragma unroll
+    for (int i = 0; i < kVecMax; ++i) {
+        const int v = i * kSlotOutThreads + tid;
+        c[i] = v < nvec ? cv[v] : make_uint4(0u, 0u, 0u, 0u);
+    }
+    const uint32_t raw = count[b];
+    const uint32_t mine = min(raw, X);
+    if (raw > X) {
         atomicOr(&flags->overflow, 2ull);
-#pragma unroll
-        for (int i = 0; i < kVec; ++i) cv[i] = c[i];
-    }
-    const uint32_t incl = wave_incl_sum(sum);
-    if (lane == kWave - 1) wtot[wv] = incl;
-    __syncthreads();
-    uint32_t run = incl - sum;
-    for (int i = 0; i < wv; ++i) run += wtot[i];
-    uint4 *ov = reinterpret_cast<uint4 *>(out) + tid * kVec;
-#pragma unroll
-    for (int i = 0; i < kVec; ++i) {
-        uint4 o;
-        o.x = run; run += c[i].x;
-        o.y = run; run += c[i].y;
-        o.z = run; run += c[i].z;
-        o.w = run; run += c[i].w;
-        ov[i] = o;
-    }
-    if (tid == kSlotOutThreads - 1) out[kSlotBuckets] = run;
+        count[b] = mine;
+    }
+    uint32_t front = 0;
+#pragma unroll
+    for (int i = 0; i < kVecMax; ++i) front += min(c[i].x, X) + min(c[i].y, X) + min(c[i].z, X) + min(c[i].w, X);
+    front = wave_sum(front);
+    const uint32_t incl = wave_incl_sum(mine);
+    if (lane == kWave - 1) { wtot[wv] = incl; wfront[wv] = front; }
+    __syncthreads();
+    uint32_t run = incl - mine;
+#pragma unroll
+    for (int i = 0; i < kSlotOutThreads / kWave; ++i) {
+        run += wfront[i];
+        if (i < wv) run += wtot[i];
+    }
+    out[b] = run;
+    if (b == kSlotBuckets - 1) out[kSlotBuckets] = run + mine;
 }
 
 #ifdef DQ_SLOT_PHASE_TIMING
diff --git a/deltaq_amd/csrc/dq_tie_walk.h b/deltaq_amd/csrc/dq_tie_walk.h
--- /dev/null
+++ b/deltaq_amd/csrc/dq_tie_walk.h
@@ -0,0 +1,56 @@
+#pragma once
+#include <cstdint>
+
+#if defined(__HIPCC__)
+#define DQ_HD __host__ __device__
+#else
+#define DQ_HD
+#endif
+
+namespace dq {
+
+constexpr int kTieMaxRun = 4096;
+
+struct TieWord {
+    uint64_t E = 0;
+    uint64_t own = 0;
+    uint32_t tail = 0;
+    bool over = false;
+};
+
+DQ_HD inline TieWord tie_word(const uint64_t *ebits, int64_t i, int64_t nwords)
+{
+    TieWord t;
+    t.E = ebits[i];
+    const uint64_t E = t.E;
+    const uint64_t next0 = (i + 1 < nwords) ? (ebits[i + 1] & 1ull) : 0ull;
+    const uint64_t A = E | (E >> 1) | (next0 << 63);
+    const int lead = (E & 1ull) ? (E == ~0ull ? 64 : __builtin_ctzll(~E)) : 0;
+    t.own = lead >= 64 ? 0ull : (A & (~0ull << lead));
+    if (t.own >> 63 && next0) {
+        int64_t j = i + 1;
+        for (;;) {
+            const uint64_t F = j < nwords ? ebits[j] : 0ull;
+            const int c = F == ~0ull ? 64 : __builtin_ctzll(~F);
+            t.tail += (uint32_t)c;
+            if (c < 64) break;
+            if (t.tail > (uint32_t)kTieMaxRun) { t.over = true; break; }
+            ++j;
+        }
+    }
+    if (t.over) { t.tail = 0; t.own = 0; }
+    return t;
+}
+
+DQ_HD inline uint64_t tie_heads(const TieWord &t) { return t.own & ~t.E; }
+
+DQ_HD inline int tie_next_group(const TieWord &t, uint64_t *heads, uint32_t *size)
+{
+    const int b = __builtin_ctzll(*heads);
+    *heads &= *heads - 1;
+    const int run = b == 63 ? 0 : __builtin_ctzll(~(t.E >> (b + 1)));
+    *size = 1u + (uint32_t)run + (b + run == 63 ? t.tail : 0u);
+    return b;
+}
+
+}
diff --git a/deltaq_amd/csrc/dq_ties.h b/deltaq_amd/csrc/dq_ties.h
--- a/deltaq_amd/csrc/dq_ties.h
+++ b/deltaq_amd/csrc/dq_ties.h
@@ -1,9 +1,10 @@
 #pragma once
 #include "dq_onesweep.h"
+#include "dq_sa_kernels.h"
+#include "dq_tie_walk.h"
 
 namespace dq {
 
-constexpr int kTieMaxRun = 4096;
 constexpr int kTieThreads = 1024;
 
 template <typename StatusT>
@@ -46,28 +47,11 @@
     const int w = threadIdx.x >> 6;
     const int64_t i = (int64_t)blockIdx.x * kTieThreads + threadIdx.x;
 
-    uint64_t E = 0, own = 0;
-    uint32_t tail = 0;
-    bool over = false;
-    if (i < nwords) {
-        E = ebits[i];
-        const uint64_t next0 = (i + 1 < nwords) ? (ebits[i + 1] & 1ull) : 0ull;
-        const uint64_t A = E | (E >> 1) | (next0 << 63);
-        const int lead = (E & 1ull) ? (E == ~0ull ? 64 : __builtin_ctzll(~E)) : 0;
-        own = lead >= 64 ? 0ull : (A & (~0ull << lead));
-        if (own >> 63 && next0) {
-            int64_t j = i + 1;
-            for (;;) {
-                const uint64_t F = j < nwords ? ebits[j] : 0ull;
-                const int c = F == ~0ull ? 64 : __builtin_ctzll(~F);
-                tail += (uint32_t)c;
-                if (c < 64) break;
-                if (tail > (uint32_t)kTieMaxRun) { over = true; break; }
-                ++j;
-            }
-        }
-    }
-    if (over) { atomicExch(&ctr->overflow, 1ull); tail = 0; own = 0; }
+    TieWord t;
+    if (i < nwords) t = tie_word(ebits, i, nwords);
+    if (t.over) atomicExch(&ctr->overflow, 1ull);
+    const uint64_t E = t.E, own = t.own;
+    const uint32_t tail = t.tail;
     const uint32_t cnt = (uint32_t)__popcll(own) + tail;
     const uint32_t incl = wave_incl_sum(cnt);
     if (lane == kWave - 1) wave_tot[w] = incl;
@@ -135,4 +119,165 @@
     (void)n;
 }
 
-}
+constexpr int kSettleThreads = 1024;
+constexpr int kSettleWords = 8;
+constexpr int kSettleTile = kSettleThreads * kSettleWords;
+constexpr int kSettlePlaceBits = 19;
+constexpr int kSettleQueue = 8192;
+constexpr int kSettleMaxGroups = 2048;
+constexpr int kSettleMaxG = 8, kSettleLen = 32;
+static_assert(kSettleTile * 64 == 1 << kSettlePlaceBits && kSettleMaxG <= 8, "a queue entry: 19 bits of place, 3 of size - 1");
+
+inline unsigned tie_settle_grid(int64_t nwords)
+{
+    const int64_t tiles = (nwords + kSettleTile - 1) / kSettleTile;
+    return (unsigned)(tiles < 1 ? 1 : tiles < kSettleMaxGroups ? tiles : kSettleMaxGroups);
+}
+
+template <typename IdxT>
+__device__ __forceinline__ bool settle_small_group(IdxT *__restrict__ SA, const uint8_t *__restrict__ text, int64_t n, int64_t h,
+                                                   int64_t p, int g)
+{
+    if (g == 2) {
+        const int64_t a = (int64_t)SA[p], b = (int64_t)SA[p + 1];
+        if ((uint64_t)a >= (uint64_t)n || (uint64_t)b >= (uint64_t)n) return false;
+        const int c = suffix_window_cmp<kSettleLen>(text, n, h, a, b);
+        if (c > 0) { SA[p] = (IdxT)b; SA[p + 1] = (IdxT)a; }
+        return c != 0;
+    }
+    int64_t s[kSettleMaxG];
+    bool ok = true;
+#pragma unroll 1
+    for (int k = 0; k < g; ++k) {
+        s[k] = (int64_t)SA[p + k];
+        ok = ok && (uint64_t)s[k] < (uint64_t)n;
+    }
+    if (!ok) return false;
+#pragma unroll 1
+    for (int pass = 0; pass < g - 1; ++pass) {
+#pragma unroll 1
+        for (int i = 0; i < g - 1 - pass; ++i) {
+            const int c = suffix_window_cmp<kSettleLen>(text, n, h, s[i], s[i + 1]);
+            if (c == 0) ok = false;
+            if (c > 0) { const int64_t x = s[i]; s[i] = s[i + 1]; s[i + 1] = x; }
+        }
+    }
+    if (!ok) return false;
+#pragma unroll 1
+    for (int k = 0; k < g; ++k)
+        if (SA[p + k] != (IdxT)s[k]) SA[p + k] = (IdxT)s[k];
+    return true;
+}
+
+__device__ __forceinline__ int64_t settle_reserve(uint32_t emit, unsigned long long *__restrict__ out_count)
+{
+    const uint32_t incl = wave_incl_sum(emit);
+    unsigned long long base = 0;
+    if (lane_id() == kWave - 1) base = atomicAdd(out_count, (unsigned long long)incl);
+    base = __shfl(base, kWave - 1, kWave);
+    return (int64_t)base + (incl - emit);
+}
+
+template <typename IdxT>
+__global__ __launch_bounds__(kSettleThreads) void tie_settle_kernel(const uint64_t *__restrict__ ebits, int64_t nwords, int64_t n,
+                                                                    IdxT *__restrict__ SA, const uint8_t *__restrict__ text,
+                                                                    int64_t h, uint64_t *__restrict__ out_rank,
+                                                                    IdxT *__restrict__ out_suf,
+                                                                    unsigned long long *__restrict__ out_count,
+                                                                    TieCounters *__restrict__ ctr)
+{
+    __shared__ uint32_t wave_tot[kSettleThreads / kWave];
+    __shared__ uint32_t queue[kSettleQueue];
+    __shared__ uint32_t queued, more;
+    if (__hip_atomic_load(&ctr->overflow, __ATOMIC_RELAXED, __HIP_MEMORY_SCOPE_AGENT) != 0) return;
+    const int lane = lane_id();
+    uint32_t members = 0;
+    const int64_t ntiles = (nwords + kSettleTile - 1) / kSettleTile;
+    for (int64_t tile = blockIdx.x; tile < ntiles; tile += gridDim.x) {
+        const int64_t w0 = tile * kSettleTile;
+        TieWord t[kSettleWords];
+#pragma unroll
+        for (int k = 0; k < kSettleWords; ++k) {
+            const int64_t i = w0 + k * kSettleThreads + threadIdx.x;
+            if (i < nwords) t[k] = tie_word(ebits, i, nwords);
+            if (t[k].over) atomicOr(&ctr->overflow, 1ull);
+            members += (uint32_t)__popcll(t[k].own) + t[k].tail;
+        }
+        int k_at = 0;
+        uint64_t heads_at = tie_heads(t[0]);
+        for (;;) {
+            if (threadIdx.x == 0) { queued = 0; more = 0; }
+            __syncthreads();
+            bool stopped = false;
+#pragma unroll
+            for (int k = 0; k < kSettleWords; ++k) {
+                const uint32_t wl = (uint32_t)(k * kSettleThreads) + threadIdx.x;
+                const int64_t i = w0 + wl;
+                uint64_t left = 0;
+                uint32_t emit = 0;
+                uint64_t heads = stopped || k < k_at ? 0ull : k == k_at ? heads_at : tie_heads(t[k]);
+                while (heads) {
+                    uint32_t g;
+                    const uint64_t before = heads;
+                    const int b = tie_next_group(t[k], &heads, &g);
+                    const int64_t p = i * 64 + b;
+                    if (p + (int64_t)g > n) { atomicOr(&ctr->overflow, 1ull); continue; }
+                    if (g <= (uint32_t)kSettleMaxG) {
+                        const uint32_t slot = atomicAdd(&queued, 1u);
+                        if (slot >= (uint32_t)kSettleQueue) { stopped = true; k_at = k; heads_at = before; break; }
+                        queue[slot] = ((g - 1u) << kSettlePlaceBits) | (wl << 6) | (uint32_t)b;
+                        continue;
+                    }
+                    left |= 1ull << b;
+                    emit += g;
+                }
+                if (__ballot(emit != 0) == 0) continue;
+                int64_t o = settle_reserve(emit, out_count);
+                while (left) {
+                    uint32_t g;
+                    const int b = tie_next_group(t[k], &left, &g);
+                    const int64_t p = i * 64 + b;
+                    for (uint32_t m = 0; m < g; ++m, ++o) {
+                        out_rank[o] = (uint64_t)p;
+                        out_suf[o] = SA[p + m];
+                    }
+                }
+            }
+            if (stopped) more = 1;
+            else k_at = kSettleWords;
+            __syncthreads();
+            const uint32_t qn = queued < (uint32_t)kSettleQueue ? queued : (uint32_t)kSettleQueue;
+            const bool again = more != 0;
+            for (uint32_t q0 = 0; q0 < qn; q0 += kSettleThreads) {
+                const uint32_t q = q0 + threadIdx.x;
+                uint32_t emit = 0;
+                int64_t p = 0;
+                if (q < qn) {
+                    const uint32_t e = queue[q];
+                    const int g = (int)(e >> kSettlePlaceBits) + 1;
+                    p = w0 * 64 + (int64_t)(e & ((1u << kSettlePlaceBits) - 1u));
+                    if (!settle_small_group<IdxT>(SA, text, n, h, p, g)) emit = (uint32_t)g;
+                }
+                if (__ballot(emit != 0) == 0) continue;
+                int64_t o = settle_reserve(emit, out_count);
+                for (uint32_t m = 0; m < emit; ++m, ++o) {
+                    out_rank[o] = (uint64_t)p;
+                    out_suf[o] = SA[p + m];
+                }
+            }
+            __syncthreads();
+            if (!again) break;
+        }
+    }
+    const uint32_t ws = wave_sum(members);
+    if (lane == 0) wave_tot[threadIdx.x >> 6] = ws;
+    __syncthreads();
+    if (threadIdx.x == 0) {
+        unsigned long long tot = 0;
+#pragma unroll
+        for (int k = 0; k < kSettleThreads / kWave; ++k) tot += wave_tot[k];
+        if (tot) atomicAdd(&ctr->count, tot);
+    }
+}
+
+}
```
